# brown-palm/goal-force

Measured on AMD Instinct MI355X. Metric: frames_per_sec (81-frame video / (50-step denoise loop + VAE decode), Wan2.2-I2V-A14B 832x480x81f), higher is better.
Workload: dtype bf16

## Files before the change

### goal_force_amd/csrc/gf_attention.hip

```cpp
#include "gf_common.h"
#include <cstdlib>
#include <type_traits>

namespace {

constexpr int QB = 256;
constexpr int KVB = 64;
constexpr int HD = 128;
constexpr int KV_TILE_BYTES = KVB * HD * 2;

constexpr int K3_RING = 2;
constexpr int K3_DMA0 = 10;
constexpr int K3_DMAS = 8;

struct AttnArgs {
    const u16* q;
    const u16* k;
    const u16* v;
    u16* o;
    int q_len, kv_len, heads, n_qblocks;
    long q_stride, k_stride, v_stride, o_stride;
    float scale_log2e;
    unsigned long long* dbg;
    float* lse;
    const u16* vt;
    long kv_pad;
    float last_key_bias;
};

constexpr int AT2_THREADS = 512;
constexpr int AT2_V_BASE = 2 * KV_TILE_BYTES;
constexpr int AT2_LDS = 4 * KV_TILE_BYTES;

template <int I, int N, class F>
__device__ __forceinline__ void static_for(F&& f) {
    if constexpr (I < N) {
        f(std::integral_constant<int, I>{});
        static_for<I + 1, N>(f);
    }
}
__device__ __forceinline__ void mfma32(f32x16& acc, const bf16x8& a, const bf16x8& b) {
    acc = __builtin_amdgcn_mfma_f32_32x32x16_bf16(a, b, acc, 0, 0, 0);
}

template <bool VT>
__global__ __launch_bounds__(AT2_THREADS, 2) void flash_attn_fwd_kernel2(const AttnArgs p) {
    extern __shared__ __attribute__((aligned(16))) char smem[];
    GF_LDS char* lds = (GF_LDS char*)smem;
    const int tid = threadIdx.x;
    const int lane = tid & 63;
    const int wave = __builtin_amdgcn_readfirstlane(tid >> 6);
    const int r = lane & 31, h = lane >> 5;
    int head, qb;
    {
        const int pid = blockIdx.x;
        if ((p.heads & 7) == 0) {
            const int xcd = pid & 7, idx = pid >> 3;
            head = xcd + 8 * (idx / p.n_qblocks);
            qb = idx % p.n_qblocks;
        } else {
            head = pid / p.n_qblocks;
            qb = pid % p.n_qblocks;
        }
    }
    const int q0 = qb * QB + wave * 32;

    bf16x8 qf[8];
    {
        const int qr = min(q0 + r, p.q_len - 1);
        const u16* qp = p.q + (long)qr * p.q_stride + head * HD + 8 * h;
#pragma unroll
        for (int kd = 0; kd < 8; ++kd) qf[kd] = *reinterpret_cast<const bf16x8*>(qp + 16 * kd);
    }

    const int dma_r = lane >> 4;
    unsigned dma_off[2][2];
#pragma unroll
    for (int jj = 0; jj < 2; ++jj) {
        const int j = 2 * wave + jj;
        const int row = 4 * j + dma_r;
        const int lch = (lane & 15) ^ ((dma_r << 2) | (j & 3));
        dma_off[jj][0] = (unsigned)row * (unsigned)p.k_stride + head * HD + lch * 8;
        dma_off[jj][1] = (unsigned)row * (unsigned)p.v_stride + head * HD + lch * 8;
    }
    const unsigned kstep = KVB * (unsigned)p.k_stride, vstep = KVB * (unsigned)p.v_stride;
    auto dma16 = [&](const u16* g, GF_LDS char* l) {
        unsigned keep;
        const unsigned dst = __builtin_amdgcn_readfirstlane((unsigned)(unsigned long)l);
        asm volatile("s_mov_b32 %0, m0\n\ts_mov_b32 m0, %2\n\ts_nop 0\n\tglobal_load_lds_dwordx4 %1, off\n\ts_mov_b32 m0, %0"
                     : "=&s"(keep)
                     : "v"(g), "s"(dst)
                     : "memory");
    };
    typedef __attribute__((ext_vector_type(4))) unsigned u32x4s;
    auto make_srd = [](const void* base) {
        const unsigned long b = (unsigned long)base;
        u32x4s r;
        r[0] = (unsigned)b;
        r[1] = (unsigned)(b >> 32) & 0xffffu;
        r[2] = 0xffffffffu;
        r[3] = 0x00020000u;
        return r;
    };
    const u32x4s srd_k = make_srd(p.k), srd_v = make_srd(VT ? (const void*)p.vt : (const void*)p.v);
    auto dma16b = [&](const u32x4s& srd, unsigned voff_bytes, unsigned soff_bytes, GF_LDS char* l) {
        unsigned keep;
        const unsigned dst = __builtin_amdgcn_readfirstlane((unsigned)(unsigned long)l);
        asm volatile("s_mov_b32 %0, m0\n\ts_mov_b32 m0, %3\n\ts_nop 0\n\tbuffer_load_dwordx4 %1, %2, %4 offen lds\n\ts_mov_b32 m0, %0"
                     : "=&s"(keep)
                     : "v"(voff_bytes), "s"(srd), "s"(dst), "s"(soff_bytes)
// ... 286 lines not shown
        __syncthreads();
    };

    stage(0, 0, 0);
    if (nt > 1) stage(0, 1, 1);
    asm volatile("s_waitcnt vmcnt(0)" ::: "memory");
    __syncthreads();
    qk_plain(C0{});
    __syncthreads();
    if (nt > 2) stage(0, 2, 0);
    stage(1, 0, 0);
    if (nt > 1) qk_plain(C1{});
    softmax_plain(C0{}, 0);
    asm volatile("s_waitcnt vmcnt(0)" ::: "memory");
    __syncthreads();
    int pi = 1;
    for (; pi + 1 <= nt - 2; pi += 2) {
        phase(C1{}, pi);
        phase(C0{}, pi + 1);
    }
    if (pi <= nt - 2) {
        phase(C1{}, pi);
        ++pi;
    }
    if (nt >= 2) {
        const int par = (nt - 1) & 1;
        stage(1, nt - 1, par);
        apply_pending();
        if (par) {
            pv_plain(C0{});
            softmax_plain(C1{}, nt - 1);
        } else {
            pv_plain(C1{});
            softmax_plain(C0{}, nt - 1);
        }
        asm volatile("s_waitcnt vmcnt(0)" ::: "memory");
        __syncthreads();
    }
    apply_pending();
    if ((nt - 1) & 1)
        pv_plain(C1{});
    else
        pv_plain(C0{});

    {
        const float l_tot = l_run + __shfl_xor(l_run, 32);
        const float inv = 1.0f / l_tot;
        const int qrow = q0 + r;
        if (p.lse && h == 0 && qrow < p.q_len) p.lse[(long)qrow * p.heads + head] = m_run * c + __builtin_amdgcn_logf(l_tot);
        __syncthreads();
        GF_LDS char* ob = lds + wave * 8192;
#pragma unroll
        for (int d = 0; d < 4; ++d)
#pragma unroll
            for (int rg = 0; rg < 4; ++rg) {
                u32x2 pk;
                pk[0] = pack2bf(oacc[d][4 * rg + 0] * inv, oacc[d][4 * rg + 1] * inv);
                pk[1] = pack2bf(oacc[d][4 * rg + 2] * inv, oacc[d][4 * rg + 3] * inv);
                *(GF_LDS u32x2*)(ob + r * 256 + (((4 * d + rg) ^ (r & 15)) << 4) + 8 * h) = pk;
            }
        asm volatile("s_waitcnt lgkmcnt(0)" ::: "memory");
#pragma unroll
        for (int it = 0; it < 8; ++it) {
            const int row = 4 * it + (lane >> 4), ch = lane & 15;
            const u16x8 v8 = *(GF_LDS u16x8*)(ob + row * 256 + ((ch ^ (row & 15)) << 4));
            if (q0 + row < p.q_len)
                *reinterpret_cast<u16x8*>(p.o + (long)(q0 + row) * p.o_stride + head * HD + 8 * ch) = v8;
        }
    }
}

constexpr int K3_NQ = 2;
template <int NQ> struct At3 {
    static constexpr int WAVES = 16 / NQ, THREADS = 64 * WAVES, ROWS = 16 * NQ, PIECES = NQ;
    static constexpr int SLOTS = 32 * NQ;
};
constexpr int AT3_V_BASE = 2 * KV_TILE_BYTES;
constexpr int AT3_LDS = 4 * KV_TILE_BYTES;

__device__ __forceinline__ void mfma16(f32x4& acc, const bf16x8& a, const bf16x8& b) {
    acc = __builtin_amdgcn_mfma_f32_16x16x32_bf16(a, b, acc, 0, 0, 0);
}

template <int NQ>
__global__ __launch_bounds__(At3<NQ>::THREADS, (NQ == 2 ? 2 : 1)) void flash_attn_fwd_kernel3(const AttnArgs p) {
    constexpr int NP = At3<NQ>::PIECES, NW = At3<NQ>::WAVES, RW = At3<NQ>::ROWS, NS = At3<NQ>::SLOTS;
    extern __shared__ __attribute__((aligned(16))) char smem[];
    GF_LDS char* lds = (GF_LDS char*)smem;
    const int tid = threadIdx.x;
    const int lane = tid & 63;
    const int wave = __builtin_amdgcn_readfirstlane(tid >> 6);
    const int r = lane & 15, g = lane >> 4;
    int head, qb0;
    {
        const int pid = blockIdx.x;
        if ((p.heads & 7) == 0) {
            const int xcd = pid & 7, idx = pid >> 3;
            head = xcd + 8 * (idx / p.n_qblocks);
            qb0 = idx % p.n_qblocks;
        } else {
            head = pid / p.n_qblocks;
            qb0 = pid % p.n_qblocks;
        }
    }
    const int q0 = qb0 * QB + wave * RW;

    bf16x8 qf[NQ][4];
#pragma unroll
    for (int qb = 0; qb < NQ; ++qb) {
        const int qr = min(q0 + 16 * qb + r, p.q_len - 1);
        const u16* qp = p.q + (long)qr * p.q_stride + head * HD + 8 * g;
#pragma unroll
        for (int ks = 0; ks < 4; ++ks) {
            qf[qb][ks] = *reinterpret_cast<const bf16x8*>(qp + 32 * ks);
        }
    }

    const int dma_r = lane >> 4;
    unsigned k_off0, vt_off0;
    {
        const int row = 4 * wave + dma_r;
        const int lch = (lane & 15) ^ (row & 15);
        k_off0 = ((unsigned)row * (unsigned)p.k_stride + head * HD + lch * 8) * 2u;
        const int vrow = 8 * wave + (lane >> 3);
        const int vch = (lane & 7) ^ ((vrow >> 1) & 7);
        vt_off0 = (unsigned)(((long)head * HD + vrow) * p.kv_pad + vch * 8) * 2u;
    }
    const unsigned kstep = KVB * (unsigned)p.k_stride * 2u;
    const unsigned k_piece = 4u * NW * (unsigned)p.k_stride * 2u, vt_piece = 8u * NW * (unsigned)p.kv_pad * 2u;
    typedef __attribute__((ext_vector_type(4))) unsigned u32x4s;
    auto make_srd = [](const void* base) {
        const unsigned long b = (unsigned long)base;
        u32x4s s;
        s[0] = (unsigned)b;
        s[1] = (unsigned)(b >> 32) & 0xffffu;
        s[2] = 0xffffffffu;
        s[3] = 0x00020000u;
        return s;
    };
    const u32x4s srd_v = make_srd(p.vt);
    auto dma16b = [&](const u32x4s& srd, unsigned voff_bytes, unsigned soff_bytes, GF_LDS char* l) __attribute__((always_inline)) {
        const unsigned dst = __builtin_amdgcn_readfirstlane((unsigned)(unsigned long)l);
        asm volatile("s_mov_b32 m0, %2\n\ts_nop 0\n\tbuffer_load_dwordx4 %0, %1, %3 offen lds"
                     :
                     : "v"(voff_bytes), "s"(srd), "s"(dst), "s"(soff_bytes)
                     : "memory");
    };
    auto srd_k_tile = [&](int t) __attribute__((always_inline)) {
        const unsigned long bb = (unsigned long)p.k + (unsigned long)(unsigned)t * kstep;
        const int rem = p.kv_len - t * KVB;
        u32x4s sd;
        sd[0] = (unsigned)bb;
        sd[1] = (unsigned)(bb >> 32) & 0xffffu;
        sd[2] = rem > 0 ? (unsigned)rem * (unsigned)p.k_stride * 2u : 0u;
        sd[3] = 0x00020000u;
        return sd;
    };
    auto stage_piece = [&](int which, int t, int buf, int jj) __attribute__((always_inline)) {
        GF_LDS char* base = lds + which * AT3_V_BASE + buf * KV_TILE_BYTES + (NW * jj + wave) * 1024;
        if (which)
            dma16b(srd_v, vt_off0, (unsigned)t * (KVB * 2u) + (unsigned)jj * vt_piece, base);
        else
            dma16b(srd_k_tile(t), k_off0, (unsigned)jj * k_piece, base);
    };
    auto stage = [&](int which, int t, int buf) __attribute__((always_inline)) {
#pragma unroll
        for (int jj = 0; jj < NP; ++jj) stage_piece(which, t, buf, jj);
    };
// ... 152 lines not shown
        if constexpr (F < 16) {
            constexpr int kk = F >> 3, db = F & 7;
            fr[F % RING] = *(GF_LDS bf16x8*)(lds + voff[kk] + db * 2048 + (1 - PAR) * KV_TILE_BYTES);
        } else if constexpr (F < 32) {
            constexpr int ks = (F - 16) >> 2, kb = (F - 16) & 3;
            fr[F % RING] = *(GF_LDS bf16x8*)(lds + koff[ks] + kb * 4096 + (1 - PAR) * KV_TILE_BYTES);
        }
    };
    auto mfma_op = [&](auto s_c, auto par_c) __attribute__((always_inline)) {
        constexpr int S = decltype(s_c)::value, PAR = decltype(par_c)::value;
        constexpr int F = S / NQ, qb = (F & 1) ? NQ - 1 - S % NQ : S % NQ;
        if constexpr (F < 16) {
            constexpr int kk = F >> 3, db = F & 7;
            mfma_pv(oacc[db][qb], fr[F % RING], pf(kk, qb));
        } else {
            constexpr int ks = (F - 16) >> 2, kb = (F - 16) & 3;
            if constexpr (ks == 0) {
                mfma_qk_first(sc[1 - PAR][kb][qb], fr[F % RING], qf[qb][ks], negm[qb]);
            } else {
                mfma_qk(sc[1 - PAR][kb][qb], fr[F % RING], qf[qb][ks]);
            }
        }
    };
    auto dma_slot = [&](auto s_c, auto par_c, int pidx) __attribute__((always_inline)) {
        constexpr int S = decltype(s_c)::value, PAR = decltype(par_c)::value;
        if constexpr (S >= K3_DMA0 && (S - K3_DMA0) % K3_DMAS == 0 && (S - K3_DMA0) / K3_DMAS < 2 * NP) {
            constexpr int i = (S - K3_DMA0) / K3_DMAS;
            if constexpr (i < NP) {
                stage_piece(1, pidx, PAR, i);
            } else {
                stage_piece(0, pidx + 2, PAR, i - NP);
            }
        }
    };
    auto phase = [&](auto par_c, int pidx) __attribute__((always_inline)) {
        constexpr int PAR = decltype(par_c)::value;
        apply_pending();
        static_for<0, RING - 1>([&](auto f_c) { frag_load(f_c, par_c); });
        float mx[NQ];
#pragma unroll
        for (int qb = 0; qb < NQ; ++qb) mx[qb] = -INFINITY;
        static_for<0, 4 * NQ>([&](auto s_c) {
            constexpr int S = decltype(s_c)::value;
            mfma_op(s_c, par_c);
            if constexpr (S % NQ == 0) frag_load(std::integral_constant<int, S / NQ + RING - 1>{}, par_c);
            {
                constexpr int kb = S / NQ, qb = S % NQ;
                const f32x4& v = sc[PAR][kb][qb];
                mx[qb] = fmaxf(fmaxf(mx[qb], v[0]), v[1]);
                mx[qb] = fmaxf(fmaxf(mx[qb], v[2]), v[3]);
            }
            __builtin_amdgcn_sched_barrier(0);
        });
        new_max(par_c, mx, false);
        float pe[2];
        static_for<4 * NQ, NS>([&](auto s_c) {
            constexpr int S = decltype(s_c)::value;
            mfma_op(s_c, par_c);
            if constexpr (S == 8 * NQ - 1 || S == 16 * NQ - 1) {
#pragma unroll
                for (int qb = 0; qb < NQ; ++qb) mfma_pv(oacc[NDB - 1][qb], ones, pf(S / (8 * NQ), qb));
            }
            if constexpr (S % NQ == 0) frag_load(std::integral_constant<int, S / NQ + RING - 1>{}, par_c);
            dma_slot(s_c, par_c, pidx);
            if constexpr (S >= 8 * NQ) {
                constexpr int T = (S - 8 * NQ) % 3, e = ((S - 8 * NQ) / 3) * 2 + (T == 2 ? 1 : T);
                constexpr int kk = e / (8 * NQ), qb = (e >> 3) % NQ, kb = 2 * kk + ((e >> 2) & 1), j = e & 3;
                if constexpr (T != 2) {
                    asm volatile("v_exp_f32 %0, %1" : "=v"(pe[T]) : "v"(sc[PAR][kb][qb][j]));
                } else {
                    unsigned w;
                    asm volatile("v_cvt_pk_bf16_f32 %0, %1, %2" : "=v"(w) : "v"(pe[0]), "v"(pe[1]));
                    pfw[kk][qb][(kb & 1) * 2 + (j >> 1)] = w;
                }
            }
            __builtin_amdgcn_sched_barrier(0);
        });
        asm volatile("s_waitcnt vmcnt(0)" ::: "memory");
        __syncthreads();
    };

    stage(0, 0, 0);
    if (nt > 1) stage(0, 1, 1);
#pragma unroll
    for (int qb = 0; qb < NQ; ++qb)
#pragma unroll
        for (int ks = 0; ks < 4; ++ks)
#pragma unroll
            for (int e = 0; e < 8; ++e) qf[qb][ks][e] = (__bf16)((float)qf[qb][ks][e] * p.scale_log2e);
    asm volatile("s_waitcnt vmcnt(0)" ::: "memory");
    __syncthreads();
    qk_plain(C0{});
    __syncthreads();
    if (nt > 2) stage(0, 2, 0);
    stage(1, 0, 0);
    softmax_plain(C0{}, 0);
    if (nt > 1) qk_plain(C1{});
    asm volatile("s_waitcnt vmcnt(0)" ::: "memory");
    __syncthreads();
    int pi = 1;
    for (; pi + 1 <= nt - 2; pi += 2) {
        phase(C1{}, pi);
        phase(C0{}, pi + 1);
    }
    if (pi <= nt - 2) {
        phase(C1{}, pi);
        ++pi;
    }
    if (nt >= 2) {
        const int par = (nt - 1) & 1;
        stage(1, nt - 1, par);
        apply_pending();
        if (par) {
            pv_plain(C0{});
            softmax_plain(C1{}, nt - 1);
        } else {
            pv_plain(C1{});
            softmax_plain(C0{}, nt - 1);
        }
        asm volatile("s_waitcnt vmcnt(0)" ::: "memory");
        __syncthreads();
    }
    apply_pending();
    if ((nt - 1) & 1)
        pv_plain(C1{});
    else
        pv_plain(C0{});

    {
        float inv[NQ];
#pragma unroll
        for (int qb = 0; qb < NQ; ++qb) {
            const float l = __shfl(oacc[NDB - 1][qb][0], r);
            inv[qb] = 1.0f / l;
            const int qrow = q0 + 16 * qb + r;
            if (p.lse && g == 0 && qrow < p.q_len) p.lse[(long)qrow * p.heads + head] = -negm[qb][0] + __builtin_amdgcn_logf(l);
        }
        __syncthreads();
        GF_LDS char* ob = lds + wave * (RW * 256);
#pragma unroll
        for (int qb = 0; qb < NQ; ++qb)
#pragma unroll
            for (int db = 0; db < 8; ++db) {
                u32x2 pk;
                pk[0] = pack2bf(oacc[db][qb][0] * inv[qb], oacc[db][qb][1] * inv[qb]);
                pk[1] = pack2bf(oacc[db][qb][2] * inv[qb], oacc[db][qb][3] * inv[qb]);
                const int row = 16 * qb + r;
                *(GF_LDS u32x2*)(ob + row * 256 + (((2 * db + (g >> 1)) ^ (row & 15)) << 4) + 8 * (g & 1)) = pk;
            }
        asm volatile("s_waitcnt lgkmcnt(0)" ::: "memory");
#pragma unroll
        for (int it = 0; it < RW / 4; ++it) {
            const int row = 4 * it + (lane >> 4), ch = lane & 15;
            const u16x8 v8 = *(GF_LDS u16x8*)(ob + row * 256 + ((ch ^ (row & 15)) << 4));
            if (q0 + row < p.q_len)
                *reinterpret_cast<u16x8*>(p.o + (long)(q0 + row) * p.o_stride + head * HD + 8 * ch) = v8;
        }
    }
}

__global__ __launch_bounds__(256) void transpose_v32_kernel(const u16* __restrict__ v, u16* __restrict__ vt, int kv_len, long kv_pad,
                                                            long v_stride) {
    __shared__ u16 tile[KVB][HD + 8];
    const int t0 = blockIdx.x * KVB, head = blockIdx.y, tid = threadIdx.x;
#pragma unroll
    for (int it = 0; it < 4; ++it) {
// ... 96 lines not shown
    a.n_qblocks = (int)((q_len + QB - 1) / QB);
    a.q_stride = q_stride;
    a.k_stride = k_stride;
    a.v_stride = v_stride;
    a.o_stride = o_stride;
    a.scale_log2e = scale * 1.4426950408889634f;
    a.lse = lse;
    a.vt = (const u16*)vt;
    a.kv_pad = kv_pad;
    a.last_key_bias = 0.f;
    if (last_key_multiplicity != 1.0f) {
        GF_CHECK_ARG(last_key_multiplicity >= 1.0f && !vt && scale > 0.f,
                     "gf_flash_attn_fwd_lastmult: multiplicity >= 1, plain-V form only (not the V^T form)");
        a.last_key_bias = log2f(last_key_multiplicity) / a.scale_log2e;
    }
    a.dbg = nullptr;
    if (vt)
        hipLaunchKernelGGL(flash_attn_fwd_kernel2<true>, dim3((unsigned)(a.n_qblocks * a.heads)), dim3(AT2_THREADS), AT2_LDS,
                           (hipStream_t)stream, a);
    else
        hipLaunchKernelGGL(flash_attn_fwd_kernel2<false>, dim3((unsigned)(a.n_qblocks * a.heads)), dim3(AT2_THREADS), AT2_LDS,
                           (hipStream_t)stream, a);
    GF_CHECK_LAUNCH("gf_flash_attn_fwd");
    return GF_OK;
}

extern "C" GF_API int gf_flash_attn_fwd(const void* q, const void* k, const void* v, void* o, int64_t q_len, int64_t kv_len,
                                 int64_t heads, int64_t head_dim, int64_t q_stride, int64_t k_stride,
                                 int64_t v_stride, int64_t o_stride, float scale, void* stream) {
    return flash_attn_fwd_impl(q, k, v, o, nullptr, q_len, kv_len, heads, head_dim, q_stride, k_stride, v_stride, o_stride, scale,
                               stream);
}

extern "C" GF_API int gf_flash_attn_fwd_lastmult(const void* q, const void* k, const void* v, void* o, int64_t q_len, int64_t kv_len,
                                                  int64_t heads, int64_t head_dim, int64_t q_stride, int64_t k_stride, int64_t v_stride,
                                                  int64_t o_stride, float scale, float last_key_multiplicity, void* stream) {
    return flash_attn_fwd_impl(q, k, v, o, nullptr, q_len, kv_len, heads, head_dim, q_stride, k_stride, v_stride, o_stride, scale,
                               stream, nullptr, 0, last_key_multiplicity);
}

extern "C" GF_API int gf_flash_attn_fwd_lse(const void* q, const void* k, const void* v, void* o, float* lse, int64_t q_len,
                                     int64_t kv_len, int64_t heads, int64_t head_dim, int64_t q_stride, int64_t k_stride,
                                     int64_t v_stride, int64_t o_stride, float scale, void* stream) {
    GF_CHECK_ARG(lse, "gf_flash_attn_fwd_lse: null lse");
    return flash_attn_fwd_impl(q, k, v, o, lse, q_len, kv_len, heads, head_dim, q_stride, k_stride, v_stride, o_stride, scale,
                               stream);
}

extern "C" GF_API int gf_transpose_v(const void* v, int64_t v_stride, void* vt, int64_t kv_len, int64_t kv_pad, int64_t heads,
                                     void* stream) {
    GF_CHECK_ARG(v && vt, "gf_transpose_v: null pointer");
    GF_CHECK_ARG(kv_len > 0 && heads > 0 && kv_pad >= kv_len && kv_pad % KVB == 0 && v_stride % 8 == 0 && v_stride >= heads * HD,
                 "gf_transpose_v: kv_pad must be a multiple of 64 covering kv_len; v_stride must cover heads*128");
    GF_CHECK_ARG(gf_aligned16(v) && gf_aligned16(vt), "gf_transpose_v: 16-byte alignment required");
    GF_CHECK_ARG(heads * HD * kv_pad < (1LL << 31), "gf_transpose_v: heads*128*kv_pad must stay below 2^31 elements");
    hipLaunchKernelGGL(transpose_v_kernel, dim3((unsigned)(kv_pad / KVB), (unsigned)heads), dim3(256), 0, (hipStream_t)stream,
                       (const u16*)v, (u16*)vt, (int)kv_len, (long)kv_pad, (long)v_stride);
    GF_CHECK_LAUNCH("gf_transpose_v");
    return GF_OK;
}

extern "C" GF_API int gf_flash_attn_fwd_vt(const void* q, const void* k, const void* vt, void* o, float* lse, int64_t q_len,
                                           int64_t kv_len, int64_t kv_pad, int64_t heads, int64_t head_dim, int64_t q_stride,
                                           int64_t k_stride, int64_t o_stride, float scale, void* stream) {
    GF_CHECK_ARG(vt && kv_pad >= kv_len && kv_pad % KVB == 0 && gf_aligned16(vt), "gf_flash_attn_fwd_vt: bad V^T buffer");
    GF_CHECK_ARG(heads * HD * kv_pad < (1LL << 31), "gf_flash_attn_fwd_vt: heads*128*kv_pad must stay below 2^31 elements");
    return flash_attn_fwd_impl(q, k, k, o, lse, q_len, kv_len, heads, head_dim, q_stride, k_stride, k_stride, o_stride, scale,
                               stream, vt, kv_pad);
}

extern "C" GF_API int gf_transpose_v32(const void* v, int64_t v_stride, void* vt, int64_t kv_len, int64_t kv_pad, int64_t heads,
                                       void* stream) {
    GF_CHECK_ARG(v && vt, "gf_transpose_v32: null pointer");
    GF_CHECK_ARG(kv_len > 0 && heads > 0 && kv_pad >= kv_len && kv_pad % KVB == 0 && v_stride % 8 == 0 && v_stride >= heads * HD,
                 "gf_transpose_v32: kv_pad must be a multiple of 64 covering kv_len; v_stride must cover heads*128");
    GF_CHECK_ARG(gf_aligned16(v) && gf_aligned16(vt), "gf_transpose_v32: 16-byte alignment required");
    GF_CHECK_ARG(heads * HD * kv_pad < (1LL << 31), "gf_transpose_v32: heads*128*kv_pad must stay below 2^31 elements");
    hipLaunchKernelGGL(transpose_v32_kernel, dim3((unsigned)(kv_pad / KVB), (unsigned)heads), dim3(256), 0, (hipStream_t)stream,
                       (const u16*)v, (u16*)vt, (int)kv_len, (long)kv_pad, (long)v_stride);
    GF_CHECK_LAUNCH("gf_transpose_v32");
    return GF_OK;
}

extern "C" GF_API int gf_flash_attn_fwd_vt32(const void* q, const void* k, const void* vt, void* o, float* lse, int64_t q_len,
                                             int64_t kv_len, int64_t kv_pad, int64_t heads, int64_t head_dim, int64_t q_stride,
                                             int64_t k_stride, int64_t o_stride, float scale, void* stream) {
    GF_CHECK_ARG(q && k && vt && o, "gf_flash_attn_fwd_vt32: null pointer");
    if (head_dim != HD) {
        gf_set_error("gf_flash_attn_fwd_vt32: head_dim=%ld unsupported (kernel is built for 128)", (long)head_dim);
        return GF_ERR_UNSUPPORTED;
    }
    GF_CHECK_ARG(q_len >= 0 && kv_len >= 2 * KVB && heads > 0 && q_len < (1 << 30) && kv_len < (1 << 30),
                 "gf_flash_attn_fwd_vt32: bad lengths q=%ld kv=%ld heads=%ld (kv_len >= 128)", (long)q_len, (long)kv_len, (long)heads);
    GF_CHECK_ARG(kv_pad >= kv_len && kv_pad % KVB == 0 && heads * HD * kv_pad < (1LL << 31), "gf_flash_attn_fwd_vt32: bad V^T buffer");
    GF_CHECK_ARG(q_stride % 8 == 0 && k_stride % 8 == 0 && o_stride % 4 == 0 && q_stride >= heads * HD && k_stride >= heads * HD &&
                     o_stride >= heads * HD,
                 "gf_flash_attn_fwd_vt32: strides must cover heads*128 and be multiples of 8");
    GF_CHECK_ARG(gf_aligned16(q) && gf_aligned16(k) && gf_aligned16(vt) && gf_aligned16(o),
                 "gf_flash_attn_fwd_vt32: 16-byte alignment required");
    GF_CHECK_ARG((kv_len + 64) * k_stride < (1LL << 31), "gf_flash_attn_fwd_vt32: kv_len*stride must stay below 2^31 elements");
    if (q_len == 0) return GF_OK;
    static GfDeviceOnce once;
    hipError_t e = gf_once_per_device(once, [] {
        return hipFuncSetAttribute(reinterpret_cast<const void*>(flash_attn_fwd_kernel3<K3_NQ>),
                                   hipFuncAttributeMaxDynamicSharedMemorySize, AT3_LDS);
    });
    if (e != hipSuccess) {
        gf_set_error("gf_flash_attn_fwd_vt32: hipFuncSetAttribute failed: %s", hipGetErrorString(e));
        return GF_ERR_LAUNCH;
    }
    AttnArgs a;
    a.q = (const u16*)q;
    a.k = (const u16*)k;
    a.v = (const u16*)k;
    a.o = (u16*)o;
    a.q_len = (int)q_len;
    a.kv_len = (int)kv_len;
    a.heads = (int)heads;
    a.n_qblocks = (int)((q_len + QB - 1) / QB);
    a.q_stride = q_stride;
    a.k_stride = k_stride;
    a.v_stride = k_stride;
    a.o_stride = o_stride;
    a.scale_log2e = scale * 1.4426950408889634f;
    a.lse = lse;
    a.vt = (const u16*)vt;
    a.kv_pad = kv_pad;
    a.dbg = nullptr;
    a.last_key_bias = 0.f;
    hipLaunchKernelGGL(flash_attn_fwd_kernel3<K3_NQ>, dim3((unsigned)(a.n_qblocks * a.heads)), dim3(At3<K3_NQ>::THREADS), AT3_LDS,
                       (hipStream_t)stream, a);
    GF_CHECK_LAUNCH("gf_flash_attn_fwd_vt32");
    return GF_OK;
}
```

### goal_force_amd/csrc/gf_cross_fold.hip

```cpp
#include "gf_common.h"

namespace {

constexpr int CF_HD = 128;
constexpr int CF_MAXK = 64;
constexpr int CF_THREADS = 256;
constexpr int CF_QB = 128;

__device__ __forceinline__ void cf_mfma32(f32x16& acc, const bf16x8& a, const bf16x8& b) {
    acc = __builtin_amdgcn_mfma_f32_32x32x16_bf16(a, b, acc, 0, 0, 0);
}

__global__ __launch_bounds__(CF_THREADS) void cross_probs_kernel(const u16* __restrict__ q, const u16* __restrict__ k, u16* __restrict__ pout,
                                                                 int q_len, int n_keys, int n_pad, int heads, long q_stride, long k_stride,
                                                                 long p_stride, float c, float last_key_bias) {
    __shared__ __attribute__((aligned(16))) char lds[CF_MAXK * 256];
    const int tid = threadIdx.x;
    const int lane = tid & 63, wave = tid >> 6;
    const int r = lane & 31, h = lane >> 5;
    const int head = blockIdx.y;
    const int q0 = blockIdx.x * CF_QB + wave * 32;
    const int halves = n_keys > 32 ? 2 : 1;

#pragma unroll
    for (int i = 0; i < (CF_MAXK * 16) / CF_THREADS; ++i) {
        const int idx = tid + CF_THREADS * i;
        const int row = idx >> 4, ch = idx & 15;
        u16x8 v8 = {0, 0, 0, 0, 0, 0, 0, 0};
        if (row < n_keys) v8 = *reinterpret_cast<const u16x8*>(k + (long)row * k_stride + head * CF_HD + ch * 8);
        const int sk = ((row & 3) << 2) | ((row >> 2) & 3);
        *(u16x8*)(lds + row * 256 + ((ch ^ sk) << 4)) = v8;
    }

    bf16x8 qf[8];
    {
        const int qr = min(q0 + r, q_len - 1);
        const u16* qp = q + (long)qr * q_stride + head * CF_HD + 8 * h;
#pragma unroll
        for (int kd = 0; kd < 8; ++kd) qf[kd] = *reinterpret_cast<const bf16x8*>(qp + 16 * kd);
    }
    __syncthreads();

    f32x16 sc[2];
#pragma unroll
    for (int e = 0; e < 16; ++e) {
        sc[0][e] = 0.f;
        sc[1][e] = 0.f;
    }
    const int sK = ((r & 3) << 2) | ((r >> 2) & 3);
#pragma unroll
    for (int kd = 0; kd < 8; ++kd) {
        const int off = 256 * r + 16 * ((2 * kd + h) ^ sK);
        cf_mfma32(sc[0], *(const bf16x8*)(lds + off), qf[kd]);
        if (halves == 2) cf_mfma32(sc[1], *(const bf16x8*)(lds + off + 32 * 256), qf[kd]);
    }

#pragma unroll
    for (int e = 0; e < 16; ++e) {
        const int key = 4 * h + (e & 3) + 8 * (e >> 2);
        if (key >= n_keys) sc[0][e] = -INFINITY;
        if (key + 32 >= n_keys) sc[1][e] = -INFINITY;
        if (key == n_keys - 1) sc[0][e] += last_key_bias;
        if (key + 32 == n_keys - 1) sc[1][e] += last_key_bias;
    }
    float mx = sc[0][0];
#pragma unroll
    for (int e = 1; e < 16; ++e) mx = fmaxf(mx, sc[0][e]);
#pragma unroll
    for (int e = 0; e < 16; ++e) mx = fmaxf(mx, sc[1][e]);
    mx = fmaxf(mx, __shfl_xor(mx, 32));
    const float mc = mx * c;
    float rs = 0.f;
#pragma unroll
    for (int e = 0; e < 16; ++e) {
        sc[0][e] = __builtin_amdgcn_exp2f(__builtin_fmaf(sc[0][e], c, -mc));
        sc[1][e] = __builtin_amdgcn_exp2f(__builtin_fmaf(sc[1][e], c, -mc));
        rs += sc[0][e] + sc[1][e];
    }
    const float l_tot = rs + __shfl_xor(rs, 32);
    const float inv = 1.0f / l_tot;
    float pl = 0.f;
#pragma unroll
    for (int e = 0; e < 16; ++e) {
        const int key = 4 * h + (e & 3) + 8 * (e >> 2);
        if (key == n_keys - 1) pl = sc[0][e];
        if (key + 32 == n_keys - 1) pl = sc[1][e];
    }
    pl += __shfl_xor(pl, 32);
    const float wl = pl * inv;
    const float wl_lo = wl - bf2f(f2bf(wl));

    const int qrow = q0 + r;
    if (qrow < q_len) {
        u16* prow = pout + (long)qrow * p_stride + (long)head * n_pad;
#pragma unroll
        for (int half = 0; half < 2; ++half)
#pragma unroll
            for (int g = 0; g < 4; ++g) {
                const int key = 32 * half + 8 * g + 4 * h;
                if (key < n_pad) {
                    float w4[4];
#pragma unroll
                    for (int i = 0; i < 4; ++i) w4[i] = key + i == n_keys ? wl_lo : sc[half][4 * g + i] * inv;
                    u32x2 pk;
                    pk[0] = pack2bf(w4[0], w4[1]);
                    pk[1] = pack2bf(w4[2], w4[3]);
                    *reinterpret_cast<u32x2*>(prow + key) = pk;
                }
            }
    }
}

constexpr int CFT_ROWS = 64;
__global__ __launch_bounds__(CF_THREADS) void cross_fold_table_kernel(const u16* __restrict__ v, const u16* __restrict__ w, u16* __restrict__ u,
                                                                      int n_keys, int n_pad, int n_out, long v_stride, long w_stride,
                                                                      long u_stride) {
    __shared__ __attribute__((aligned(16))) u16 vs[CF_MAXK * CF_HD];
    const int tid = threadIdx.x;
    const int head = blockIdx.y;
    for (int idx = tid; idx < n_pad * 16; idx += CF_THREADS) {
        const int row = idx >> 4, ch = idx & 15;
        u16x8 v8 = {0, 0, 0, 0, 0, 0, 0, 0};
        if (row <= n_keys) v8 = *reinterpret_cast<const u16x8*>(v + (long)min(row, n_keys - 1) * v_stride + head * CF_HD + ch * 8);
        *reinterpret_cast<u16x8*>(vs + row * CF_HD + ch * 8) = v8;
    }
    __syncthreads();
    const int n = blockIdx.x * CFT_ROWS + (tid >> 2), jg = tid & 3;
    if (n >= n_out) return;
    const int nj = n_pad >> 2;
    float acc[CF_MAXK / 4];
#pragma unroll
    for (int i = 0; i < CF_MAXK / 4; ++i) acc[i] = 0.f;
    const u16* wr = w + (long)n * w_stride + head * CF_HD;
    for (int d0 = 0; d0 < CF_HD; d0 += 8) {
        const u16x8 w8 = *reinterpret_cast<const u16x8*>(wr + d0);
        float wf[8];
#pragma unroll
        for (int e = 0; e < 8; ++e) wf[e] = bf2f(w8[e]);
#pragma unroll
        for (int i = 0; i < CF_MAXK / 4; ++i) {
            if (i < nj) {
                const u16x8 v8 = *reinterpret_cast<const u16x8*>(vs + (jg + 4 * i) * CF_HD + d0);
#pragma unroll
                for (int e = 0; e < 8; ++e) acc[i] = __builtin_fmaf(bf2f(v8[e]), wf[e], acc[i]);
            }
        }
    }
    u16* ur = u + (long)n * u_stride + (long)head * n_pad;
#pragma unroll
    for (int i = 0; i < CF_MAXK / 4; ++i) {
        const int j = jg + 4 * i;
        if (i < nj) ur[j] = j <= n_keys ? f2bf(acc[i]) : (u16)0;
    }
}

}

extern "C" GF_API int gf_cross_probs(const void* q, const void* k, void* p, int64_t q_len, int64_t n_keys, int64_t n_pad, int64_t heads,
                                     int64_t head_dim, int64_t q_stride, int64_t k_stride, int64_t p_stride, float scale,
                                     float last_key_multiplicity, void* stream) {
    GF_CHECK_ARG(q && k && p, "gf_cross_probs: null pointer");
    if (head_dim != CF_HD) {
        gf_set_error("gf_cross_probs: head_dim=%ld unsupported (kernel is built for 128)", (long)head_dim);
        return GF_ERR_UNSUPPORTED;
    }
    GF_CHECK_ARG(q_len >= 0 && q_len < (1 << 30) && heads > 0 && heads < 65536, "gf_cross_probs: bad sizes q=%ld heads=%ld", (long)q_len,
                 (long)heads);
    GF_CHECK_ARG(n_keys >= 1 && n_pad % 16 == 0 && n_pad > n_keys && n_pad <= CF_MAXK,
                 "gf_cross_probs: 1 <= n_keys=%ld < n_pad=%ld <= 64, n_pad a multiple of 16", (long)n_keys, (long)n_pad);
    GF_CHECK_ARG(q_stride % 8 == 0 && k_stride % 8 == 0 && p_stride % 4 == 0 && q_stride >= heads * CF_HD && k_stride >= heads * CF_HD &&
                     p_stride >= heads * n_pad,
                 "gf_cross_probs: strides must cover the rows (q, k: multiples of 8; p: of 4, >= heads * n_pad)");
    GF_CHECK_ARG(gf_aligned16(q) && gf_aligned16(k) && ((uintptr_t)p & 7u) == 0, "gf_cross_probs: alignment (q, k 16 bytes, p 8 bytes)");
    GF_CHECK_ARG(scale > 0.f && last_key_multiplicity >= 1.0f, "gf_cross_probs: scale > 0, multiplicity >= 1");
    if (q_len == 0) return GF_OK;
    const float c = scale * 1.4426950408889634f;
    const float bias = last_key_multiplicity != 1.0f ? log2f(last_key_multiplicity) / c : 0.f;
    const dim3 grid((unsigned)((q_len + CF_QB - 1) / CF_QB), (unsigned)heads);
    hipLaunchKernelGGL(cross_probs_kernel, grid, dim3(CF_THREADS), 0, (hipStream_t)stream, (const u16*)q, (const u16*)k, (u16*)p,
                       (int)q_len, (int)n_keys, (int)n_pad, (int)heads, (long)q_stride, (long)k_stride, (long)p_stride, c, bias);
    GF_CHECK_LAUNCH("gf_cross_probs");
    return GF_OK;
}

extern "C" GF_API int gf_cross_fold_table(const void* v, const void* w_o, void* u, int64_t n_keys, int64_t n_pad, int64_t heads,
                                          int64_t head_dim, int64_t n_out, int64_t v_stride, int64_t w_stride, int64_t u_stride,
                                          void* stream) {
    GF_CHECK_ARG(v && w_o && u, "gf_cross_fold_table: null pointer");
    if (head_dim != CF_HD) {
        gf_set_error("gf_cross_fold_table: head_dim=%ld unsupported (kernel is built for 128)", (long)head_dim);
        return GF_ERR_UNSUPPORTED;
    }
    GF_CHECK_ARG(heads > 0 && heads < 65536 && n_out > 0 && n_out < (1 << 30), "gf_cross_fold_table: bad sizes heads=%ld N=%ld", (long)heads,
                 (long)n_out);
    GF_CHECK_ARG(n_keys >= 1 && n_pad % 16 == 0 && n_pad > n_keys && n_pad <= CF_MAXK,
                 "gf_cross_fold_table: 1 <= n_keys=%ld < n_pad=%ld <= 64, n_pad a multiple of 16", (long)n_keys, (long)n_pad);
    GF_CHECK_ARG(v_stride % 8 == 0 && w_stride % 8 == 0 && v_stride >= heads * CF_HD && w_stride >= heads * CF_HD && u_stride >= heads * n_pad,
                 "gf_cross_fold_table: strides must cover the rows (v, w_o: multiples of 8; u >= heads * n_pad)");
    GF_CHECK_ARG(gf_aligned16(v) && gf_aligned16(w_o) && ((uintptr_t)u & 1u) == 0, "gf_cross_fold_table: alignment");
    const dim3 grid((unsigned)((n_out + CFT_ROWS - 1) / CFT_ROWS), (unsigned)heads);
    hipLaunchKernelGGL(cross_fold_table_kernel, grid, dim3(CF_THREADS), 0, (hipStream_t)stream, (const u16*)v, (const u16*)w_o, (u16*)u,
                       (int)n_keys, (int)n_pad, (int)n_out, (long)v_stride, (long)w_stride, (long)u_stride);
    GF_CHECK_LAUNCH("gf_cross_fold_table");
    return GF_OK;
}
```

### goal_force_amd/csrc/gf_gemm.hip

```cpp
#include "gf_common.h"
#include <cstdlib>
#include <type_traits>


namespace {

constexpr int BM = 256, BN = 256, BK = 64;
constexpr int GEMM_THREADS = 512;
constexpr int TILE_BYTES = BM * BK * 2;
constexpr int STAGE_BYTES = 2 * TILE_BYTES;
constexpr int GEMM_LDS = 2 * STAGE_BYTES;
constexpr int GROUP_M = 8;

struct ConvGeom {
    const u16* src;
    const u16* cache;
    const u16* zero;
    int H, W, C, Ho, Wo, kt, ks, mode, t_stride, t_off, taps;
    int hist_front;
    int c64;
    long frame;
    float inv_c, inv_ks2;
};

struct GemmArgs {
    const u16* A;
    const u16* W;
    const u16* bias;
    u16* C;
    const u16* R;
    const u16* gate;
    const float* row_scale;
    int M, N, K;
    long lda, ldw, ldc, ldr;
    long sA = 0, sW = 0, sC = 0;
    int tiles_m, tiles_n;
    unsigned long long* rsv0 = nullptr;
    ConvGeom cv;
    int rsv1 = 0;
    int stagger;
    int wrows;
    int stagger_rows;
    int group_m;
    int rsv2 = 0;
};

constexpr int GF_EPI_VT32 = 6;

__device__ __forceinline__ void glds16(const void* g, GF_LDS char* l) {
    __builtin_amdgcn_global_load_lds((const GF_GLOBAL void*)g, (GF_LDS void*)l, 16, 0, 0);
}

typedef __attribute__((ext_vector_type(8))) int i32x8;

template <int EPI>
__device__ __forceinline__ float gf_epi_act(float lin) {
    if constexpr (EPI == GF_EPI_BIAS_GELU_TANH) return gelu_tanh_f(rbf(lin));
    else if constexpr (EPI == GF_EPI_BIAS_SILU) {
        const float y = rbf(lin);
        return y / (1.0f + expf(-y));
    } else return lin;
}

template <int EPI, bool FP8>
__global__ __launch_bounds__(GEMM_THREADS, 2) void gemm_kernel(const GemmArgs p) {
    static_assert(FP8, "only the fp8 form of this kernel ships (launch_gemm); bf16 with M < 512 runs gemm_ph_kernel");
    constexpr int ESZ = FP8 ? 1 : 2;
    constexpr int BKE = 128 / ESZ;
    extern __shared__ __attribute__((aligned(16))) char smem[];
    GF_LDS char* lds = (GF_LDS char*)smem;

    const int tid = threadIdx.x;
    const int lane = tid & 63;
    const int wave = __builtin_amdgcn_readfirstlane(tid >> 6);

    const int nwg = p.tiles_m * p.tiles_n;
    int v;
    {
        const int pid = blockIdx.x;
        const int xcd = pid & 7, local = pid >> 3;
        const int q = nwg >> 3, r = nwg & 7;
        v = (xcd < r ? xcd * (q + 1) : r * (q + 1) + (xcd - r) * q) + local;
    }
    const int per_group = GROUP_M * p.tiles_n;
    const int group = v / per_group;
    const int first_m = group * GROUP_M;
    const int gsz = min(p.tiles_m - first_m, GROUP_M);
    const int in_group = v - group * per_group;
    const int tile_m = first_m + in_group % gsz;
    const int tile_n = in_group / gsz;
    const int m0 = tile_m * BM, n0 = tile_n * BN;

    const int srow = lane >> 3;
    const int schunk = (lane & 7) ^ srow;
    const char* a_src[4];
    const char* b_src[4];
#pragma unroll
    for (int i = 0; i < 4; ++i) {
        const int row = (wave * 4 + i) * 8 + srow;
        const int am = min(m0 + row, p.M - 1);
        const int bn = min(n0 + row, p.N - 1);
        a_src[i] = (const char*)p.A + ((long)am * p.lda) * ESZ + schunk * 16;
        b_src[i] = (const char*)p.W + ((long)bn * p.ldw) * ESZ + schunk * 16;
    }
    auto stage = [&](int buf, int kt) {
        GF_LDS char* sa = lds + buf * STAGE_BYTES + wave * 4096;
        GF_LDS char* sb = sa + TILE_BYTES;
        const int koff = kt * 128;
#pragma unroll
        for (int i = 0; i < 4; ++i) {
            glds16(a_src[i] + koff, sa + i * 1024);
            glds16(b_src[i] + koff, sb + i * 1024);
        }
    };

    const int wm = wave >> 2, wn = wave & 3;
    const int frow = lane & 15;
    const int fq = lane >> 4;
    const int sw = frow & 7;
    const int a_base = (wm * 128 + frow) * 128;
    const int b_base = TILE_BYTES + (wn * 64 + frow) * 128;
    const int ch0 = ((0 * 4 + fq) ^ sw) << 4;
    const int ch1 = ((1 * 4 + fq) ^ sw) << 4;

    f32x4 acc[8][4];
#pragma unroll
    for (int i = 0; i < 8; ++i)
#pragma unroll
        for (int j = 0; j < 4; ++j) acc[i][j] = f32x4{0.f, 0.f, 0.f, 0.f};

// ... 605 lines not shown
#pragma unroll
        for (int it = 0; it < 32; ++it) {
            const int mr = m0 + wm * 128 + it * 4 + (lane >> 4);
            if (mr < p.M && nr < p.N) {
                rres[it] = __builtin_nontemporal_load(reinterpret_cast<const u16x8*>(p.R + (long)mr * p.ldr + nr));
            } else {
                rres[it] = u16x8{0, 0, 0, 0, 0, 0, 0, 0};
            }
        }
    }
    f32x4 csc[(FP8 && EPI == GF_EPI_VT32) ? 8 : 1];
    if constexpr (FP8 && EPI == GF_EPI_VT32) {
#pragma unroll
        for (int j = 0; j < 8; ++j) {
            const int n = n0 + wn * 128 + j * 16 + fq * 4;
#pragma unroll
            for (int r = 0; r < 4; ++r) csc[j][r] = (n + r < p.wrows) ? p.row_scale[n + r] : 0.f;
        }
    }
    a4_static_for<0, 8>([&](auto j_c) {
        constexpr int j = decltype(j_c)::value;
        const int n = n0 + wn * 128 + j * 16 + fq * 4;
        const float bv[4] = {bf2f(bpre[j][0]), bf2f(bpre[j][1]), bf2f(bpre[j][2]), bf2f(bpre[j][3])};
        a4_static_for<0, 8>([&](auto i_c) {
            constexpr int i = decltype(i_c)::value;
            constexpr int A0 = (i * 8 + j) * 4;
            float y[4] = {a4_acc<A0>(), a4_acc<A0 + 1>(), a4_acc<A0 + 2>(), a4_acc<A0 + 3>()};
            if constexpr (FP8 && EPI != GF_EPI_VT32) {
#pragma unroll
                for (int r = 0; r < 4; ++r) y[r] = y[r] * rsc[i] + bv[r];
            }
            if constexpr (EPI == GF_EPI_VT32) {
                const float bm = bf2f(bpre[i][0]);
                if constexpr (FP8) {
#pragma unroll
                    for (int r = 0; r < 4; ++r) y[r] = (n + r < p.wrows) ? y[r] * csc[j][r] + bm : 0.f;
                } else {
#pragma unroll
                    for (int r = 0; r < 4; ++r) y[r] = (n + r < p.wrows) ? y[r] + bm : 0.f;
                }
            } else if constexpr (EPI == GF_EPI_BIAS_GELU_TANH) {
                const unsigned l01 = FP8 ? pack2bf(y[0], y[1]) : pack2bf(y[0] + bv[0], y[1] + bv[1]);
                const unsigned l23 = FP8 ? pack2bf(y[2], y[3]) : pack2bf(y[2] + bv[2], y[3] + bv[3]);
                gf_f32x2 g01 = {__uint_as_float(l01 << 16), __uint_as_float(l01 & 0xffff0000u)};
                gf_f32x2 g23 = {__uint_as_float(l23 << 16), __uint_as_float(l23 & 0xffff0000u)};
                gelu_tanh_f4(g01, g23);
                y[0] = g01[0];
                y[1] = g01[1];
                y[2] = g23[0];
                y[3] = g23[1];
            } else {
#pragma unroll
                for (int r = 0; r < 4; ++r) {
                    y[r] = gf_epi_act<EPI>(FP8 ? y[r] : y[r] + bv[r]);
                }
            }
            u32x2 pk;
            pk[0] = pack2bf(y[0], y[1]);
            pk[1] = pack2bf(y[2], y[3]);
            const int row = i * 16 + frow;
            const int slot = (j * 4 + fq) ^ ((row & 15) << 1);
            *(GF_LDS u32x2*)(ep + row * 256 + slot * 8) = pk;
        });
    });
    asm volatile("s_waitcnt lgkmcnt(0)" ::: "memory");
    {
        const int cc = lane & 15;
        const int n = n0 + wn * 128 + cc * 8;
        const bool n_ok = n < p.N;
        const u16x8 g8 = gpre;
#pragma unroll
        for (int it = 0; it < 32; ++it) {
            const int row = it * 4 + (lane >> 4);
            const int m = m0 + wm * 128 + row;
            u16x8 yv;
            if constexpr (EPI == GF_EPI_VT32) {
                const int G = cc >> 2, g = cc & 3, sw = (row & 15) << 1;
                const u16x4 lo = *(GF_LDS u16x4*)(ep + row * 256 + (((8 * G + g) ^ sw) << 3));
                const u16x4 hi = *(GF_LDS u16x4*)(ep + row * 256 + (((8 * G + 4 + g) ^ sw) << 3));
                yv = u16x8{lo[0], lo[1], lo[2], lo[3], hi[0], hi[1], hi[2], hi[3]};
            } else {
                yv = *(GF_LDS u16x8*)(ep + row * 256 + ((cc ^ (row & 15)) << 4));
            }
            if (m < p.M && n_ok) {
                u16x8 o = yv;
                if constexpr (HAS_R) {
                    const u16x8 r8 = rres[it];
#pragma unroll
                    for (int e = 0; e < 8; ++e) {
                        float t = bf2f(yv[e]);
                        if (EPI == GF_EPI_BIAS_GATE_RESID) t = rbf(bf2f(g8[e]) * t);
                        o[e] = (EPI == GF_EPI_BIAS_MUL) ? f2bf(t * bf2f(r8[e]))
                                                        : f2bf(bf2f(r8[e]) + t);
                    }
                }
                __builtin_nontemporal_store(o, reinterpret_cast<u16x8*>(p.C + (long)m * p.ldc + n));
            }
        }
    }
}

template <int EPI, bool FP8 = false>
int launch_gemm_a4(const GemmArgs& a0, hipStream_t stream) {
    GemmArgs a = a0;
    {
        const int g = gf_options().a4_group_m.load(std::memory_order_relaxed);
        a.group_m = g > 0 ? g : (a.K * (FP8 ? 1 : 2) >= 16384 ? 4 : GROUP_M);
    }
    static GfDeviceOnce once;
    hipError_t e = gf_once_per_device(once, [] {
        return hipFuncSetAttribute(reinterpret_cast<const void*>(gemm_a4_kernel<EPI, FP8>),
                                   hipFuncAttributeMaxDynamicSharedMemorySize, GEMM_LDS);
    });
    if (e != hipSuccess) {
        gf_set_error("gf_gemm: hipFuncSetAttribute(%d B LDS) failed: %s", GEMM_LDS, hipGetErrorString(e));
        return GF_ERR_LAUNCH;
    }
    hipLaunchKernelGGL((gemm_a4_kernel<EPI, FP8>), dim3((unsigned)(a.tiles_m * a.tiles_n)), dim3(A4_THREADS), GEMM_LDS, stream, a);
    GF_CHECK_LAUNCH(FP8 ? "gf_gemm_fp8" : "gf_gemm_bf16");
    return GF_OK;
}

template <int EPI, bool FP8>
int launch_gemm(const GemmArgs& a, hipStream_t stream) {
    const bool use_a4 = gf_options().prefer_8wave.load(std::memory_order_relaxed) == 0;
    if constexpr (!FP8) {
        if (use_a4 && a.M >= 512 && a.K % 64 == 0 && 256L * a.lda * 2 + a.K * 2L < (1L << 31) &&
            256L * a.ldw * 2 + a.K * 2L < (1L << 31))
            return launch_gemm_a4<EPI>(a, stream);
    } else {
        if (use_a4 && a.M >= 512 && a.K % 128 == 0 && 256L * a.lda + a.K < (1L << 31) && 256L * a.ldw + a.K < (1L << 31))
            return launch_gemm_a4<EPI, true>(a, stream);
    }
    static GfDeviceOnce once;
    hipError_t e = gf_once_per_device(once, [] {
        const void* fn;
        if constexpr (FP8) fn = reinterpret_cast<const void*>(gemm_kernel<EPI, true>);
        else fn = reinterpret_cast<const void*>(gemm_ph_kernel<EPI, false>);
        return hipFuncSetAttribute(fn, hipFuncAttributeMaxDynamicSharedMemorySize, GEMM_LDS);
    });
    if (e != hipSuccess) {
        gf_set_error("gf_gemm: hipFuncSetAttribute(%d B LDS) failed: %s", GEMM_LDS, hipGetErrorString(e));
        return GF_ERR_LAUNCH;
    }
    if constexpr (FP8)
        hipLaunchKernelGGL((gemm_kernel<EPI, true>), dim3((unsigned)(a.tiles_m * a.tiles_n)), dim3(GEMM_THREADS), GEMM_LDS, stream, a);
    else
        hipLaunchKernelGGL((gemm_ph_kernel<EPI, false>), dim3((unsigned)(a.tiles_m * a.tiles_n)), dim3(GEMM_THREADS), GEMM_LDS,
                           stream, a);
    GF_CHECK_LAUNCH(FP8 ? "gf_gemm_fp8" : "gf_gemm_bf16");
    return GF_OK;
}

template <int EPI, int NB, int CONV>
int launch_conv(const GemmArgs& a, hipStream_t stream, int batch = 1) {
    static GfDeviceOnce once;
    hipError_t e = gf_once_per_device(once, [] {
        return hipFuncSetAttribute(reinterpret_cast<const void*>(gemm_ph_kernel<EPI, false, CONV, NB>),
                                   hipFuncAttributeMaxDynamicSharedMemorySize, GEMM_LDS);
    });
    if (e != hipSuccess) {
        gf_set_error("gf_conv3d: hipFuncSetAttribute(%d B LDS) failed: %s", GEMM_LDS, hipGetErrorString(e));
        return GF_ERR_LAUNCH;
    }
    hipLaunchKernelGGL((gemm_ph_kernel<EPI, false, CONV, NB>), dim3((unsigned)(a.tiles_m * a.tiles_n), (unsigned)batch), dim3(GEMM_THREADS),
                       GEMM_LDS, stream, a);
    GF_CHECK_LAUNCH("gf_conv3d_bf16");
    return GF_OK;
}

}
__device__ __attribute__((used, visibility("default"))) u16 gf_conv_zero_page[128] = {};
namespace {

const u16* conv_zero_page() {
    static GfDeviceOnce once;
    static const u16* page[64] = {};
    int dev = 0;
    if (hipGetDevice(&dev) != hipSuccess || dev < 0 || dev >= 64) return nullptr;
    hipError_t e = gf_once_per_device(once, [dev] {
        void* z = nullptr;
        hipError_t r = hipGetSymbolAddress(&z, HIP_SYMBOL(gf_conv_zero_page));
        if (r == hipSuccess) page[dev] = (const u16*)z;
        return r;
    });
    return e == hipSuccess ? page[dev] : nullptr;
}

}

static int gemm_dispatch(bool fp8, const void* A, int64_t lda, const void* W, int64_t ldw, const float* row_scale,
                         const void* bias, void* C, int64_t ldc, int64_t M, int64_t N, int64_t K, int epilogue,
                         const void* resid, int64_t ldr, const void* gate, void* stream) {
    const char* fn = fp8 ? "gf_gemm_fp8" : "gf_gemm_bf16";
    const int bke = fp8 ? 128 : 64, lal = fp8 ? 16 : 8;
    GF_CHECK_ARG(A && W && C, "%s: null A/W/C", fn);
    GF_CHECK_ARG(M >= 0 && N > 0 && K > 0, "%s: bad sizes M=%ld N=%ld K=%ld", fn, (long)M, (long)N, (long)K);
    GF_CHECK_ARG(K % bke == 0, "%s: K=%ld must be a multiple of %d", fn, (long)K, bke);
    GF_CHECK_ARG(N % 8 == 0, "%s: N=%ld must be a multiple of 8", fn, (long)N);
    GF_CHECK_ARG(lda % lal == 0 && ldw % lal == 0 && ldc % 8 == 0 && lda >= K && ldw >= K && ldc >= N,
                 "%s: leading dimensions must be multiples of %d (A/W) / 8 (C) and cover the row", fn, lal);
    GF_CHECK_ARG(gf_aligned16(A) && gf_aligned16(W) && gf_aligned16(C) && (!bias || gf_aligned16(bias)),
                 "%s: 16-byte alignment required", fn);
    GF_CHECK_ARG(M < (1 << 30) && N < (1 << 30), "%s: M/N too large", fn);
    GF_CHECK_ARG(!fp8 || row_scale, "%s: row_scale is required", fn);
    const bool need_r = epilogue == GF_EPI_BIAS_GATE_RESID || epilogue == GF_EPI_BIAS_RESID || epilogue == GF_EPI_BIAS_MUL;
    GF_CHECK_ARG(!need_r || (resid && ldr % 8 == 0 && ldr >= N && gf_aligned16(resid)),
                 "%s: residual epilogue needs an aligned resid with ldr >= N", fn);
    GF_CHECK_ARG(epilogue != GF_EPI_BIAS_GATE_RESID || (gate && gf_aligned16(gate)),
                 "%s: gate epilogue needs an aligned gate vector", fn);
    if (M == 0) return GF_OK;
    GemmArgs a;
    a.A = (const u16*)A;
    a.W = (const u16*)W;
    a.bias = (const u16*)bias;
    a.C = (u16*)C;
    a.R = (const u16*)resid;
    a.gate = (const u16*)gate;
    a.row_scale = row_scale;
    a.M = (int)M;
    a.N = (int)N;
    a.K = (int)K;
    a.lda = lda;
    a.ldw = ldw;
    a.ldc = ldc;
    a.ldr = ldr;
    a.tiles_m = (int)((M + BM - 1) / BM);
    a.tiles_n = (int)((N + BN - 1) / BN);
    a.stagger = gf_options().a4_stagger.load(std::memory_order_relaxed);
    a.wrows = (int)N;
    a.stagger_rows = 0;
    hipStream_t s = (hipStream_t)stream;
#define GF_GEMM_CASE(E) case E: return fp8 ? launch_gemm<E, true>(a, s) : launch_gemm<E, false>(a, s);
    switch (epilogue) {
        GF_GEMM_CASE(GF_EPI_BIAS)
        GF_GEMM_CASE(GF_EPI_BIAS_GELU_TANH)
        GF_GEMM_CASE(GF_EPI_BIAS_GATE_RESID)
        GF_GEMM_CASE(GF_EPI_BIAS_RESID)
        GF_GEMM_CASE(GF_EPI_BIAS_SILU)
        GF_GEMM_CASE(GF_EPI_BIAS_MUL)
        default:
            gf_set_error("%s: unknown epilogue %d", fn, epilogue);
            return GF_ERR_INVALID_ARG;
    }
#undef GF_GEMM_CASE
}

extern "C" GF_API int gf_gemm_bf16(const void* A, int64_t lda, const void* W, int64_t ldw, const void* bias, void* C,
                                   int64_t ldc, int64_t M, int64_t N, int64_t K, int epilogue, const void* resid,
                                   int64_t ldr, const void* gate, void* stream) {
    return gemm_dispatch(false, A, lda, W, ldw, nullptr, bias, C, ldc, M, N, K, epilogue, resid, ldr, gate, stream);
}

extern "C" GF_API int gf_gemm_fp8(const void* A8, int64_t lda, const void* W8, int64_t ldw, const float* row_scale,
                                  const void* bias, void* C, int64_t ldc, int64_t M, int64_t N, int64_t K, int epilogue,
                                  const void* resid, int64_t ldr, const void* gate, void* stream) {
    return gemm_dispatch(true, A8, lda, W8, ldw, row_scale, bias, C, ldc, M, N, K, epilogue, resid, ldr, gate, stream);
}

extern "C" GF_API int gf_linear_vt32(const void* x, int64_t ldx, const void* w, int64_t ldw, const void* bias, void* vt,
                                     int64_t kv_len, int64_t kv_pad, int64_t N, int64_t K, void* stream) {
    GF_CHECK_ARG(x && w && vt, "gf_linear_vt32: null x/w/vt");
    GF_CHECK_ARG(kv_len > 0 && kv_pad >= kv_len && kv_pad % 64 == 0 && kv_pad - kv_len < 64, "gf_linear_vt32: kv_pad = kv_len rounded up to 64");
    GF_CHECK_ARG(N >= 512 && N % 128 == 0 && K > 0 && K % 64 == 0, "gf_linear_vt32: N=%ld (>= 512, multiple of 128), K=%ld (multiple of 64)", (long)N, (long)K);
    GF_CHECK_ARG(ldx % 8 == 0 && ldw % 8 == 0 && ldx >= K && ldw >= K, "gf_linear_vt32: leading dimensions must be multiples of 8 covering K");
    GF_CHECK_ARG(gf_aligned16(x) && gf_aligned16(w) && gf_aligned16(vt) && (!bias || ((uintptr_t)bias & 1u) == 0), "gf_linear_vt32: alignment");
    GF_CHECK_ARG(N * kv_pad < (1LL << 31) && 256L * ldx * 2 + K * 2L < (1L << 31) && 256L * ldw * 2 + K * 2L < (1L << 31),
                 "gf_linear_vt32: operand too large for 32-bit staging offsets");
    GemmArgs a;
    a.A = (const u16*)w;
    a.W = (const u16*)x;
    a.bias = (const u16*)bias;
    a.C = (u16*)vt;
    a.R = nullptr;
    a.gate = nullptr;
    a.row_scale = nullptr;
    a.M = (int)N;
    a.N = (int)kv_pad;
    a.K = (int)K;
    a.lda = ldw;
    a.ldw = ldx;
    a.ldc = kv_pad;
    a.ldr = 0;
    a.tiles_m = (int)((N + BM - 1) / BM);
    a.tiles_n = (int)((kv_pad + BN - 1) / BN);
    a.stagger = gf_options().a4_stagger.load(std::memory_order_relaxed);
    a.wrows = (int)kv_len;
    a.stagger_rows = 1;
    return launch_gemm_a4<GF_EPI_VT32>(a, (hipStream_t)stream);
}

extern "C" GF_API int gf_linear_vt32_fp8(const void* x8, int64_t ldx, const float* x_scale, const void* w8, int64_t ldw, const void* bias,
                                         void* vt, int64_t kv_len, int64_t kv_pad, int64_t N, int64_t K, void* stream) {
    GF_CHECK_ARG(x8 && w8 && vt && x_scale, "gf_linear_vt32_fp8: null x8/w8/vt/x_scale");
    GF_CHECK_ARG(kv_len > 0 && kv_pad >= kv_len && kv_pad % 64 == 0 && kv_pad - kv_len < 64, "gf_linear_vt32_fp8: kv_pad = kv_len rounded up to 64");
    GF_CHECK_ARG(N >= 512 && N % 128 == 0 && K > 0 && K % 128 == 0, "gf_linear_vt32_fp8: N=%ld (>= 512, multiple of 128), K=%ld (multiple of 128)", (long)N, (long)K);
    GF_CHECK_ARG(ldx % 16 == 0 && ldw % 16 == 0 && ldx >= K && ldw >= K, "gf_linear_vt32_fp8: leading dimensions must be multiples of 16 covering K");
    GF_CHECK_ARG(gf_aligned16(x8) && gf_aligned16(w8) && gf_aligned16(vt) && (!bias || ((uintptr_t)bias & 1u) == 0), "gf_linear_vt32_fp8: alignment");
    GF_CHECK_ARG(N * kv_pad < (1LL << 31) && 256L * ldx + K < (1L << 31) && 256L * ldw + K < (1L << 31),
                 "gf_linear_vt32_fp8: operand too large for 32-bit staging offsets");
    GemmArgs a;
    a.A = (const u16*)w8;
    a.W = (const u16*)x8;
    a.bias = (const u16*)bias;
    a.C = (u16*)vt;
    a.R = nullptr;
    a.gate = nullptr;
    a.row_scale = x_scale;
    a.M = (int)N;
    a.N = (int)kv_pad;
    a.K = (int)K;
    a.lda = ldw;
    a.ldw = ldx;
    a.ldc = kv_pad;
    a.ldr = 0;
    a.tiles_m = (int)((N + BM - 1) / BM);
    a.tiles_n = (int)((kv_pad + BN - 1) / BN);
    a.stagger = gf_options().a4_stagger.load(std::memory_order_relaxed);
    a.wrows = (int)kv_len;
    a.stagger_rows = 1;
    return launch_gemm_a4<GF_EPI_VT32, true>(a, (hipStream_t)stream);
}

extern "C" GF_API int gf_gemm_bf16_batched(const void* A, int64_t lda, int64_t strideA, const void* W, int64_t ldw, int64_t strideW,
                                           void* C, int64_t ldc, int64_t strideC, int64_t M, int64_t N, int64_t K, int64_t batch,
                                           void* stream) {
    GF_CHECK_ARG(A && W && C, "gf_gemm_bf16_batched: null A/W/C");
    GF_CHECK_ARG(M > 0 && N > 0 && K > 0 && batch > 0 && batch < 65536, "gf_gemm_bf16_batched: bad sizes");
    GF_CHECK_ARG(K % 64 == 0 && N % 8 == 0, "gf_gemm_bf16_batched: K=%ld must be a multiple of 64 and N=%ld of 8", (long)K, (long)N);
    GF_CHECK_ARG(lda >= K && ldw >= K && ldc >= N && lda % 8 == 0 && ldw % 8 == 0 && ldc % 8 == 0 && strideA % 8 == 0 && strideW % 8 == 0 &&
                     strideC % 8 == 0 && strideA >= 0 && strideW >= 0 && strideC >= 0,
                 "gf_gemm_bf16_batched: leading dimensions / strides must be multiples of 8 elements covering K / N");
    GF_CHECK_ARG(gf_aligned16(A) && gf_aligned16(W) && gf_aligned16(C), "gf_gemm_bf16_batched: 16-byte alignment required");
    GF_CHECK_ARG(M < (1L << 30) && N < (1L << 30), "gf_gemm_bf16_batched: M / N too large");
// ... 127 lines not shown
```

### goal_force_amd/csrc/gf_rowops.hip

```cpp
#include "gf_common.h"

namespace {

constexpr int ROW_THREADS = 128;
constexpr int ROW_NCH = 8;

__global__ __launch_bounds__(ROW_THREADS) void layernorm_modulate_kernel(
    const u16* __restrict__ x, u16* __restrict__ out, const u16* __restrict__ weight,
    const u16* __restrict__ bias, const u16* __restrict__ scale1p, const u16* __restrict__ shift,
    int dim, long x_stride, long out_stride, float eps) {
    __shared__ float red[ROW_THREADS / 64];
    const long row = blockIdx.x;
    const int tid = threadIdx.x;
    const int nchunks = dim >> 3;
    const u16* xr = x + row * x_stride;
    u16x8 v[ROW_NCH];
    float s = 0.f;
#pragma unroll
    for (int i = 0; i < ROW_NCH; ++i) {
        const int c = tid + i * ROW_THREADS;
        if (c < nchunks) {
            v[i] = *reinterpret_cast<const u16x8*>(xr + (c << 3));
#pragma unroll
            for (int j = 0; j < 8; ++j) s += bf2f(v[i][j]);
        }
    }
    const float mean = block_sum<ROW_THREADS>(s, red) / (float)dim;
    float q = 0.f;
#pragma unroll
    for (int i = 0; i < ROW_NCH; ++i) {
        const int c = tid + i * ROW_THREADS;
        if (c < nchunks) {
#pragma unroll
            for (int j = 0; j < 8; ++j) {
                const float d = bf2f(v[i][j]) - mean;
                q += d * d;
            }
        }
    }
    const float var = block_sum<ROW_THREADS>(q, red) / (float)dim;
    const float rstd = 1.0f / sqrtf(var + eps);
    u16* orow = out + row * out_stride;
#pragma unroll
    for (int i = 0; i < ROW_NCH; ++i) {
        const int c = tid + i * ROW_THREADS;
        if (c < nchunks) {
            u16x8 w8, b8, sc8, sh8;
            if (weight) w8 = *reinterpret_cast<const u16x8*>(weight + (c << 3));
            if (bias) b8 = *reinterpret_cast<const u16x8*>(bias + (c << 3));
            if (scale1p) sc8 = *reinterpret_cast<const u16x8*>(scale1p + (c << 3));
            if (shift) sh8 = *reinterpret_cast<const u16x8*>(shift + (c << 3));
            u16x8 o;
#pragma unroll
            for (int j = 0; j < 8; ++j) {
                float y = (bf2f(v[i][j]) - mean) * rstd;
                if (weight) y = y * bf2f(w8[j]);
                if (bias) y = y + bf2f(b8[j]);
                y = rbf(y);
                if (scale1p) y = rbf(y * bf2f(sc8[j]));
                if (shift) y = rbf(y + bf2f(sh8[j]));
                o[j] = f2bf(y);
            }
            *reinterpret_cast<u16x8*>(orow + (c << 3)) = o;
        }
    }
}

__global__ __launch_bounds__(ROW_THREADS) void rmsnorm_rope_kernel(
    u16* __restrict__ x, const u16* __restrict__ weight, const float* __restrict__ cos_tab,
    const float* __restrict__ sin_tab, int dim, int head_dim, long x_stride, float eps) {
    __shared__ float red[ROW_THREADS / 64];
    const long row = blockIdx.x;
    const int tid = threadIdx.x;
    const int nchunks = dim >> 3;
    u16* xr = x + row * x_stride;
    u16x8 v[ROW_NCH];
    float s = 0.f;
#pragma unroll
    for (int i = 0; i < ROW_NCH; ++i) {
        const int c = tid + i * ROW_THREADS;
        if (c < nchunks) {
            v[i] = *reinterpret_cast<const u16x8*>(xr + (c << 3));
#pragma unroll
// ... 179 lines not shown
        const float sc = fmaxf(rbf(mx / 448.0f), 1.0f);
        if (lane == 0) scale_out[row] = sc;
        const float den = sc + 1e-8f;
        const bool unit = den == 1.0f;
        unsigned char* orow = (unsigned char*)outp + row * out_stride + lane * 8;
#pragma unroll
        for (int i = 0; i < NCH; ++i) {
            unsigned w[2];
#pragma unroll
            for (int h2 = 0; h2 < 2; ++h2) {
                gf_f32x2 f0 = unpack2bf(v[i][2 * h2]), f1 = unpack2bf(v[i][2 * h2 + 1]);
                if (!unit) {
                    f0 = gf_f32x2{f0[0] / den, f0[1] / den};
                    f1 = gf_f32x2{f1[0] / den, f1[1] / den};
                }
                unsigned t = 0;
                t = __builtin_amdgcn_cvt_pk_fp8_f32(f0[0], f0[1], t, false);
                t = __builtin_amdgcn_cvt_pk_fp8_f32(f1[0], f1[1], t, true);
                w[h2] = t;
            }
            *reinterpret_cast<u32x2*>(orow + i * 512) = u32x2{w[0], w[1]};
        }
    }
}

template <int NCH, int ROPE>
__global__ __launch_bounds__(64 * WROWS) void rmsnorm_rope_wave_kernel(u16* __restrict__ x, const u16* __restrict__ weight,
                                                                         const float* __restrict__ cos_tab,
                                                                         const float* __restrict__ sin_tab, long rows,
                                                                         int head_dim, long x_stride, float eps) {
    constexpr int DIM = NCH * 512;
    const long row = (long)blockIdx.x * WROWS + (threadIdx.x >> 6);
    if (row >= rows) return;
    const int lane = threadIdx.x & 63;
    u16* xr = x + row * x_stride + lane * 8;
    u16x8 v[NCH];
    float s = 0.f;
#pragma unroll
    for (int i = 0; i < NCH; ++i) {
        v[i] = *reinterpret_cast<const u16x8*>(xr + i * 512);
#pragma unroll
        for (int j = 0; j < 8; ++j) {
            const float f = bf2f(v[i][j]);
            s += f * f;
        }
    }
    const float rstd = 1.0f / sqrtf(wave_sum(s) * (1.0f / DIM) + eps);
    const int half = head_dim >> 1;
    f32x4 cs1 = {0.f, 0.f, 0.f, 0.f}, sn1 = {0.f, 0.f, 0.f, 0.f};
    if constexpr (ROPE == 1) {
        const int p0 = ((lane * 8) % head_dim) >> 1;
        cs1 = *reinterpret_cast<const f32x4*>(cos_tab + row * half + p0);
        sn1 = *reinterpret_cast<const f32x4*>(sin_tab + row * half + p0);
    }
#pragma unroll
    for (int i = 0; i < NCH; ++i) {
        const int c0 = i * 512 + lane * 8;
        const u16x8 w8 = *reinterpret_cast<const u16x8*>(weight + c0);
        float y[8];
#pragma unroll
        for (int j = 0; j < 8; ++j) {
            const float n = rbf(bf2f(v[i][j]) * rstd);
            y[j] = rbf(n * bf2f(w8[j]));
        }
        u16x8 o;
        if constexpr (ROPE != 0) {
            f32x4 cs = cs1, sn = sn1;
            if constexpr (ROPE == 2) {
                const int p0 = (c0 % head_dim) >> 1;
                cs = *reinterpret_cast<const f32x4*>(cos_tab + row * half + p0);
                sn = *reinterpret_cast<const f32x4*>(sin_tab + row * half + p0);
            }
#pragma unroll
            for (int p = 0; p < 4; ++p) {
                const float a = y[2 * p], b = y[2 * p + 1];
                o[2 * p] = f2bf(__builtin_fmaf(a, cs[p], -(b * sn[p])));
                o[2 * p + 1] = f2bf(__builtin_fmaf(a, sn[p], b * cs[p]));
            }
        } else {
#pragma unroll
            for (int j = 0; j < 8; ++j) o[j] = f2bf(y[j]);
        }
        *reinterpret_cast<u16x8*>(xr + i * 512) = o;
    }
}

__global__ __launch_bounds__(ROW_THREADS) void quant_fp8_rowscale_kernel(const u16* __restrict__ x,
                                                                         unsigned char* __restrict__ out,
                                                                         float* __restrict__ scale, int dim,
                                                                         long x_stride, long out_stride) {
    __shared__ float red[ROW_THREADS / 64];
    const long row = blockIdx.x;
    const int tid = threadIdx.x;
    const int nchunks = dim >> 3;
    const u16* xr = x + row * x_stride;
    constexpr int NCH = 14;
    u16x8 v[NCH];
    float mx = 0.f;
#pragma unroll
    for (int i = 0; i < NCH; ++i) {
        const int c = tid + i * ROW_THREADS;
        if (c < nchunks) {
            v[i] = *reinterpret_cast<const u16x8*>(xr + (c << 3));
#pragma unroll
            for (int j = 0; j < 8; ++j) mx = fmaxf(mx, fabsf(bf2f(v[i][j])));
        }
    }
#pragma unroll
    for (int o = 32; o > 0; o >>= 1) mx = fmaxf(mx, __shfl_xor(mx, o));
    if ((tid & 63) == 0) red[tid >> 6] = mx;
    __syncthreads();
    mx = fmaxf(red[0], red[1]);
    const float sc = fmaxf(rbf(mx / 448.0f), 1.0f);
    if (tid == 0) scale[row] = sc;
    const float den = sc + 1e-8f;
    unsigned char* orow = out + row * out_stride;
#pragma unroll
    for (int i = 0; i < NCH; ++i) {
        const int c = tid + i * ROW_THREADS;
        if (c < nchunks) {
            float f[8];
#pragma unroll
            for (int j = 0; j < 8; ++j) f[j] = bf2f(v[i][j]) / den;
            unsigned w0 = 0, w1 = 0;
            w0 = __builtin_amdgcn_cvt_pk_fp8_f32(f[0], f[1], w0, false);
            w0 = __builtin_amdgcn_cvt_pk_fp8_f32(f[2], f[3], w0, true);
            w1 = __builtin_amdgcn_cvt_pk_fp8_f32(f[4], f[5], w1, false);
            w1 = __builtin_amdgcn_cvt_pk_fp8_f32(f[6], f[7], w1, true);
            *reinterpret_cast<u32x2*>(orow + (c << 3)) = u32x2{w0, w1};
        }
    }
}

template <int NCH>
__global__ __launch_bounds__(64 * WROWS) void layernorm_modulate_fp8_wave_kernel(
    const u16* __restrict__ x, unsigned char* __restrict__ out8, float* __restrict__ scale, const u16* __restrict__ weight,
    const u16* __restrict__ bias, const u16* __restrict__ scale1p, const u16* __restrict__ shift, long rows, long x_stride,
    long out_stride, float eps) {
    constexpr int DIM = NCH * 512;
    const long row = (long)blockIdx.x * WROWS + (threadIdx.x >> 6);
    if (row >= rows) return;
    const int lane = threadIdx.x & 63;
    const u16* xr = x + row * x_stride + lane * 8;
    u16x8 v[NCH];
    float s = 0.f;
#pragma unroll
    for (int i = 0; i < NCH; ++i) {
        v[i] = *reinterpret_cast<const u16x8*>(xr + i * 512);
#pragma unroll
        for (int j = 0; j < 8; ++j) s += bf2f(v[i][j]);
    }
    const float mean = wave_sum(s) * (1.0f / DIM);
    float q = 0.f;
#pragma unroll
    for (int i = 0; i < NCH; ++i)
#pragma unroll
        for (int j = 0; j < 8; ++j) {
            const float d = bf2f(v[i][j]) - mean;
            q += d * d;
        }
    const float rstd = 1.0f / sqrtf(wave_sum(q) * (1.0f / DIM) + eps);
    float mx = 0.f;
#pragma unroll
    for (int i = 0; i < NCH; ++i) {
        const int c0 = i * 512 + lane * 8;
        u16x8 w8, b8, sc8, sh8;
// ... 118 lines not shown
    hipLaunchKernelGGL(layernorm_modulate_kernel, dim3((unsigned)rows), dim3(ROW_THREADS), 0,
                       (hipStream_t)stream, (const u16*)x, (u16*)out, (const u16*)weight, (const u16*)bias,
                       (const u16*)scale1p, (const u16*)shift, (int)dim, (long)x_stride, (long)out_stride, eps);
    GF_CHECK_LAUNCH("gf_layernorm_modulate");
    return GF_OK;
}

extern "C" GF_API int gf_layernorm_modulate_fp8(const void* x, void* out8, float* scale, const void* weight, const void* bias,
                                                const void* scale1p, const void* shift, int64_t rows, int64_t dim,
                                                int64_t x_stride, int64_t out_stride, float eps, void* stream) {
    GF_CHECK_ARG(x && out8 && scale, "gf_layernorm_modulate_fp8: null x/out8/scale");
    GF_CHECK_ARG(rows >= 0 && (dim == 5120 || dim == 4096 || dim == 1536),
                 "gf_layernorm_modulate_fp8: dim=%ld is not one of the wave-per-row widths (5120, 4096, 1536); use "
                 "gf_layernorm_modulate + gf_quant_fp8_rowscale", (long)dim);
    GF_CHECK_ARG(x_stride % 8 == 0 && out_stride % 8 == 0 && gf_aligned16(x) && (((uintptr_t)out8) & 7u) == 0,
                 "gf_layernorm_modulate_fp8: rows must be 16-byte (x) / 8-byte (out8) aligned");
    GF_CHECK_ARG((!weight || gf_aligned16(weight)) && (!bias || gf_aligned16(bias)) &&
                     (!scale1p || gf_aligned16(scale1p)) && (!shift || gf_aligned16(shift)),
                 "gf_layernorm_modulate_fp8: vectors must be 16-byte aligned");
    if (rows == 0) return GF_OK;
    {
        const int mode = (!weight && !bias && !scale1p && !shift) ? 0 : (weight && bias && !scale1p && !shift) ? 1
                         : (!weight && !bias && scale1p && shift) ? 2 : -1;
        const void* av = mode == 1 ? weight : scale1p;
        const void* bv = mode == 1 ? bias : shift;
        const dim3 grid_((unsigned)((rows + WROWS - 1) / WROWS)), block_(64 * WROWS);
#define GF_LN2(NCH, M)                                                                                                   \
    if (dim == NCH * 512 && mode == M) {                                                                                 \
        hipLaunchKernelGGL((layernorm_wave2_kernel<NCH, M, true>), grid_, block_, 0, (hipStream_t)stream, (const u16*)x, out8,     \
                           scale, (const u16*)av, (const u16*)bv, (long)rows, (long)x_stride, (long)out_stride, eps);   \
        GF_CHECK_LAUNCH("gf_layernorm_modulate_fp8");                                                                    \
        return GF_OK;                                                                                                    \
    }
        GF_LN2(10, 0) GF_LN2(10, 1) GF_LN2(10, 2) GF_LN2(8, 0) GF_LN2(8, 1) GF_LN2(8, 2) GF_LN2(3, 0) GF_LN2(3, 1) GF_LN2(3, 2)
#undef GF_LN2
    }
#define GF_LN8_WAVE(NCH)                                                                                                 \
    if (dim == NCH * 512) {                                                                                              \
        hipLaunchKernelGGL(layernorm_modulate_fp8_wave_kernel<NCH>, dim3((unsigned)((rows + WROWS - 1) / WROWS)),        \
                           dim3(64 * WROWS), 0, (hipStream_t)stream, (const u16*)x, (unsigned char*)out8, scale,          \
                           (const u16*)weight, (const u16*)bias, (const u16*)scale1p, (const u16*)shift, (long)rows,     \
                           (long)x_stride, (long)out_stride, eps);                                                       \
    }
    GF_LN8_WAVE(10) GF_LN8_WAVE(8) GF_LN8_WAVE(3)
#undef GF_LN8_WAVE
    GF_CHECK_LAUNCH("gf_layernorm_modulate_fp8");
    return GF_OK;
}

extern "C" GF_API int gf_rmsnorm_rope(void* x, const void* weight, const float* cos_tab, const float* sin_tab,
                               int64_t rows, int64_t dim, int64_t head_dim, int64_t x_stride, float eps,
                               void* stream) {
    GF_CHECK_ARG(x && weight, "gf_rmsnorm_rope: null x/weight");
    GF_CHECK_ARG(rows >= 0 && dim > 0 && dim % 8 == 0 && dim <= ROW_THREADS * ROW_NCH * 8,
                 "gf_rmsnorm_rope: dim=%ld must be a multiple of 8 and <= %d", (long)dim,
                 ROW_THREADS * ROW_NCH * 8);
    GF_CHECK_ARG((cos_tab == nullptr) == (sin_tab == nullptr), "gf_rmsnorm_rope: cos/sin must both be set or both NULL");
    GF_CHECK_ARG(head_dim > 0 && head_dim % 8 == 0 && dim % head_dim == 0,
                 "gf_rmsnorm_rope: head_dim=%ld must be a multiple of 8 dividing dim", (long)head_dim);
    GF_CHECK_ARG(x_stride % 8 == 0 && gf_aligned16(x) && gf_aligned16(weight) &&
                     (!cos_tab || (gf_aligned16(cos_tab) && gf_aligned16(sin_tab))),
                 "gf_rmsnorm_rope: 16-byte alignment required");
    if (rows == 0) return GF_OK;
#define GF_RMS_WAVE_ROPE(NCH, ROPE)                                                                                      \
    if (rope_ == ROPE)                                                                                                   \
        hipLaunchKernelGGL((rmsnorm_rope_wave_kernel<NCH, ROPE>), grid_, block_, 0, (hipStream_t)stream, (u16*)x,        \
                           (const u16*)weight, cos_tab, sin_tab, (long)rows, (int)head_dim, (long)x_stride, eps);
#define GF_RMS_WAVE(NCH)                                                                                                 \
    if (dim == NCH * 512) {                                                                                              \
        const dim3 grid_((unsigned)((rows + WROWS - 1) / WROWS)), block_(64 * WROWS);                                     \
        const int rope_ = !cos_tab ? 0 : (512 % head_dim == 0 ? 1 : 2);                                                  \
        GF_RMS_WAVE_ROPE(NCH, 0) GF_RMS_WAVE_ROPE(NCH, 1) GF_RMS_WAVE_ROPE(NCH, 2)                                        \
        GF_CHECK_LAUNCH("gf_rmsnorm_rope");                                                                              \
        return GF_OK;                                                                                                    \
    }
    GF_RMS_WAVE(10) GF_RMS_WAVE(8) GF_RMS_WAVE(3)
#undef GF_RMS_WAVE
#undef GF_RMS_WAVE_ROPE
    hipLaunchKernelGGL(rmsnorm_rope_kernel, dim3((unsigned)rows), dim3(ROW_THREADS), 0, (hipStream_t)stream,
                       (u16*)x, (const u16*)weight, cos_tab, sin_tab, (int)dim, (int)head_dim, (long)x_stride, eps);
    GF_CHECK_LAUNCH("gf_rmsnorm_rope");
    return GF_OK;
}
```

### goal_force_amd/dit.py

```python
from __future__ import annotations

import math
from typing import Optional, Tuple

import torch
import torch.nn as nn

from . import ops
from ._lib import GoalForceError


def precompute_freqs_cis(dim: int, end: int = 1024, theta: float = 10000.0):
    freqs = 1.0 / (theta ** (torch.arange(0, dim, 2)[: (dim // 2)].double() / dim))
    freqs = torch.outer(torch.arange(end), freqs)
    return torch.polar(torch.ones_like(freqs), freqs)


def precompute_freqs_cis_3d(dim: int, end: int = 1024, theta: float = 10000.0):
    return (precompute_freqs_cis(dim - 2 * (dim // 3), end, theta),
            precompute_freqs_cis(dim // 3, end, theta),
            precompute_freqs_cis(dim // 3, end, theta))


class RopeTable:
# ... 29 lines not shown
def _as_rope(freqs, device) -> RopeTable:
    if isinstance(freqs, RopeTable):
        return freqs
    if torch.is_tensor(freqs) and freqs.is_complex():
        return RopeTable(freqs.detach().cpu(), device)
    raise GoalForceError("freqs must be a RopeTable or the reference's complex [S,1,d/2] tensor")


_SINUSOID_FREQS = {}


def sinusoidal_embedding_1d(dim, position):
    key = (dim, position.device)
    inv = _SINUSOID_FREQS.get(key)
    if inv is None:
        inv = torch.pow(10000, -torch.arange(dim // 2, dtype=torch.float64).div(dim // 2)).to(position.device)
        _SINUSOID_FREQS[key] = inv
    sinusoid = torch.outer(position.detach().type(torch.float64), inv)
    return torch.cat([torch.cos(sinusoid), torch.sin(sinusoid)], dim=1).to(position.dtype)


def flash_attention(q: torch.Tensor, k: torch.Tensor, v: torch.Tensor, num_heads: int, compatibility_mode=False):
    if q.dim() != 3 or k.dim() != 3 or v.dim() != 3 or not (q.shape[0] == k.shape[0] == v.shape[0]):
        raise GoalForceError("flash_attention: q, k, v must be [B, S, num_heads * head_dim] with equal B")
    return torch.stack([ops.flash_attn(q[b].contiguous(), k[b].contiguous(), v[b].contiguous(), num_heads, finished_q=True)
                        for b in range(q.shape[0])])


def modulate(x: torch.Tensor, shift: torch.Tensor, scale: torch.Tensor):
    if x.dim() == 2:
        return ops.modulate(x, shift.reshape(-1).contiguous(), scale.reshape(-1).contiguous())
    d = x.shape[-1]
    sh, sc = (t.reshape(-1, d) if t.numel() != d else t.reshape(1, d) for t in (shift, scale))
    if sh.shape[0] not in (1, x.shape[0]) or sc.shape[0] not in (1, x.shape[0]):
        raise GoalForceError("modulate: shift / scale must be [B or 1, 1, D] (per-token modulation is outside the Goal-Force path)")
    return torch.stack([ops.modulate(x[b].contiguous(), sh[b if sh.shape[0] > 1 else 0].contiguous(),
                                     sc[b if sc.shape[0] > 1 else 0].contiguous()) for b in range(x.shape[0])])


def rope_apply(x: torch.Tensor, freqs, num_heads: int):
    rope = _as_rope(freqs, x.device)
    hd = x.shape[-1] // num_heads
    return torch.stack([ops.rope_apply(x[b].contiguous(), rope.cos, rope.sin, hd) for b in range(x.shape[0])])


_CACHE_EPOCH = [0]


def invalidate_caches():
    _CACHE_EPOCH[0] += 1


def param_key(*tensors):
    return (_CACHE_EPOCH[0],) + tuple((id(t), str(t.device), t.data_ptr(), None if t.is_inference() else t._version) for t in tensors)


class QuantizedInput:

    def __init__(self, x2=None, x8=None, scale=None):
        self.x8, self.scale = ops.quant_fp8_rowscale(x2) if x2 is not None else (x8, scale)

    @classmethod
    def layernorm(cls, x2, **kw):
        return cls(None, *ops.layernorm_modulate_fp8(x2, **kw))

    @property
    def shape(self):
        return self.x8.shape

    @property
    def is_cuda(self):
        return self.x8.is_cuda


def linear(x2, lin: nn.Linear, epilogue=ops.EPI_BIAS, resid=None, gate=None, out=None):
    w8 = getattr(lin, "_gf_w8", None)
    if w8 is None:
        return ops.gemm(x2, lin.weight, lin.bias, epilogue=epilogue, resid=resid, gate=gate, out=out)
    if lin._gf_w8_key != param_key(lin.weight):
        w8 = lin._gf_w8 = ops.cast_fp8(lin.weight.detach().contiguous())
        lin._gf_w8_key = param_key(lin.weight)
    q = x2 if isinstance(x2, QuantizedInput) else QuantizedInput(x2)
    return ops.gemm_fp8(q.x8, q.scale, w8, lin.bias, epilogue=epilogue, resid=resid, gate=gate, out=out)


def enable_fp8(module: nn.Module, enabled=True):
    for blk in module.modules():
        if isinstance(blk, DiTBlock):
            for lin in blk.modules():
                if isinstance(lin, nn.Linear):
                    lin._gf_w8 = ops.cast_fp8(lin.weight.detach().contiguous()) if enabled else None
                    lin._gf_w8_key = param_key(lin.weight) if enabled else None
    return module



def enable_sage_attention(module: nn.Module, enabled=True):
    for blk in module.modules():
        if isinstance(blk, DiTBlock):
            blk.self_attn._gf_sage = bool(enabled)
    return module


def sageattn(q, k, v, tensor_layout="HND", is_causal=False, sm_scale=None, return_lse=False, **kw):
    if is_causal:
        raise GoalForceError("sageattn: is_causal=True is not supported (the Wan DiT attention is non-causal)")
    if return_lse:
        raise GoalForceError("sageattn: return_lse=True is not supported")
    if tensor_layout not in ("HND", "NHD"):
        raise GoalForceError(f"sageattn: tensor_layout {tensor_layout!r} (HND or NHD)")
    if q.dim() != 4 or k.dim() != 4 or v.dim() != 4:
        raise GoalForceError("sageattn: q, k, v must be 4-D")
    if q.shape[-1] != 128 or k.shape[-1] != 128 or v.shape[-1] != 128:
        raise GoalForceError(f"sageattn: head_dim {q.shape[-1]} is not supported (the kernel is built for 128)")
    if tensor_layout == "HND":
        q, k, v = (t.transpose(1, 2) for t in (q, k, v))
    B, sq, n, _ = q.shape
    if k.shape[0] != B or v.shape != k.shape or k.shape[2] != n:
        raise GoalForceError("sageattn: q / k / v batch, head or key counts differ")
    out = torch.empty((B, sq, n, 128), dtype=torch.bfloat16, device=q.device)
    for b in range(B):
        q2, k2, v2 = (t[b].reshape(t.shape[1], n * 128) for t in (q, k, v))
        ops.sage_attn(q2, k2, v2, n, scale=sm_scale, out=out[b].view(sq, n * 128))
    return out.transpose(1, 2) if tensor_layout == "HND" else out


def pad_run(ctx2: torch.Tensor) -> int:
    L = ctx2.shape[0]
    if L < 2:
        return max(L - 1, 0)
    differs = (ctx2[1:] != ctx2[:-1]).any(dim=1)
    idx = torch.nonzero(differs)
    return int(idx[-1]) + 1 if idx.numel() else 0


def _tokens2d(x: torch.Tensor) -> torch.Tensor:
    if x.dim() == 3:
        if x.shape[0] != 1:
            raise GoalForceError("hot-path modules take batch 1 ([1,S,D]); loop over the batch")
        return x[0]
    return x


class RMSNorm(nn.Module):

    def __init__(self, dim, eps=1e-5):
        super().__init__()
        self.eps = eps
        self.weight = nn.Parameter(torch.ones(dim))

    def forward(self, x):
        y = x.clone()
        ops.rmsnorm_rope(_tokens2d(y), self.weight, None, None, head_dim=8, eps=self.eps)
        return y


class SelfAttention(nn.Module):

    def __init__(self, dim: int, num_heads: int, eps: float = 1e-6):
        super().__init__()
        self.dim, self.num_heads, self.head_dim = dim, num_heads, dim // num_heads
        self.q, self.k, self.v, self.o = (nn.Linear(dim, dim) for _ in range(4))
        self.norm_q, self.norm_k = RMSNorm(dim, eps=eps), RMSNorm(dim, eps=eps)

    def attend(self, x2: torch.Tensor, rope: RopeTable, sp=None, keep=None) -> torch.Tensor:
        fp8 = getattr(self.q, "_gf_w8", None) is not None
        sage = getattr(self, "_gf_sage", False)
        if sage and keep is not None:
            raise GoalForceError("training through a block with enable_sage_attention is refused (the sage backend has no backward): "
                                 "call enable_sage_attention(module, False) first")
        attn = ops.sage_attn if sage else ops.flash_attn
        xin = (x2 if isinstance(x2, QuantizedInput) else QuantizedInput(x2)) if fp8 else x2
        q_cos, q_sin, attn_scale = rope.cos, rope.sin, None
        if ops._OPT["attn_q_prescale"]:
            (q_cos, q_sin), attn_scale = rope.scaled(Q_PRESCALE(self.head_dim)), math.log(2.0)
        if sp is not None and keep is None:
            k = linear(xin, self.k)
            ops.rmsnorm_rope(k, self.norm_k.weight, rope.cos, rope.sin, self.head_dim, self.norm_k.eps)
            hk = sp.heads_start(k, self.num_heads)
            hv = sp.heads_start(linear(xin, self.v), self.num_heads)
            q = linear(xin, self.q)
            ops.rmsnorm_rope(q, self.norm_q.weight, q_cos, q_sin, self.head_dim, self.norm_q.eps)
            hq = sp.heads_start(q, self.num_heads)
            return sp.attention_started(hq, hk, hv, self.num_heads, tuple(q.shape), scale=attn_scale, backend="sage" if sage else "flash")
        q, k = linear(xin, self.q), linear(xin, self.k)
        if keep is not None and keep.get("wide"):
            keep["qp"], keep["kp"] = q, k
            q, k = q.clone(), k.clone()
        ops.rmsnorm_rope(q, self.norm_q.weight, q_cos, q_sin, self.head_dim, self.norm_q.eps)
        ops.rmsnorm_rope(k, self.norm_k.weight, rope.cos, rope.sin, self.head_dim, self.norm_k.eps)
        if sp is None and keep is None and not fp8 and x2.is_cuda and self.v.weight.shape[0] >= 512 \
                and ops.vt32_ok(x2.shape[0], self.num_heads, self.head_dim):
            return attn(q, k, None, self.num_heads, vt=ops.linear_vt32(x2, self.v.weight, self.v.bias), scale=attn_scale)
        if sp is None and keep is None and fp8 and xin.is_cuda and self.v.weight.shape[0] >= 512 and self.v.weight.shape[1] % 128 == 0 \
                and ops.vt32_ok(xin.shape[0], self.num_heads, self.head_dim):
            if self.v._gf_w8_key != param_key(self.v.weight):
                self.v._gf_w8 = ops.cast_fp8(self.v.weight.detach().contiguous())
                self.v._gf_w8_key = param_key(self.v.weight)
            return attn(q, k, None, self.num_heads, vt=ops.linear_vt32_fp8(xin.x8, xin.scale, self.v._gf_w8, self.v.bias), scale=attn_scale)
        v = linear(xin, self.v)
        if sp is not None:
            return sp.attention(q, k, v, self.num_heads, scale=attn_scale, backend="sage" if sage else "flash")
        if keep is not None:
            keep["attn"], keep["lse"] = ops.flash_attn_lse(q, k, v, self.num_heads, scale=attn_scale)
            if keep.get("wide"):
                keep["v"] = v
            return keep["attn"]
        return attn(q, k, v, self.num_heads, scale=attn_scale)

    def forward(self, x, freqs):
        x2 = _tokens2d(x)
        a = self.attend(x2, _as_rope(freqs, x.device))
        return linear(a, self.o).view(x.shape)


class CrossAttention(nn.Module):

    def __init__(self, dim: int, num_heads: int, eps: float = 1e-6, has_image_input: bool = False):
        super().__init__()
        if has_image_input:
            raise NotImplementedError("has_image_input=True (CLIP image tokens) is outside the Goal-Force path")
        self.dim, self.num_heads, self.head_dim = dim, num_heads, dim // num_heads
        self.q, self.k, self.v, self.o = (nn.Linear(dim, dim) for _ in range(4))
        self.norm_q, self.norm_k = RMSNorm(dim, eps=eps), RMSNorm(dim, eps=eps)
        self.has_image_input = False

    def context_kv(self, ctx2: torch.Tensor, fold: bool = True, pad_n: Optional[int] = None):
        m = 1
        if fold and ctx2.is_cuda and ops._OPT["fold_pad_keys"]:
            n = pad_run(ctx2) if pad_n is None else pad_n
            if ctx2.shape[0] - n >= 2 and n + 1 < ops.VT_MIN_KV:
                m = ctx2.shape[0] - n
                ctx2 = ctx2[: n + 1]
        cin = QuantizedInput(ctx2) if getattr(self.k, "_gf_w8", None) is not None else ctx2
        k, v = linear(cin, self.k), linear(cin, self.v)
        ops.rmsnorm_rope(k, self.norm_k.weight, None, None, self.head_dim, self.norm_k.eps)
        return k, v, m

    def attend(self, x2, kv):
        q = linear(x2, self.q)
        ops.rmsnorm_rope(q, self.norm_q.weight, None, None, self.head_dim, self.norm_q.eps)
        return ops.flash_attn(q, kv[0], kv[1], self.num_heads, last_key_mult=kv[2] if len(kv) > 2 else 1)

    FOLD_K_MAX = 2560

    def fold_ok(self, kv) -> bool:
        if not ops._OPT["fold_cross_o"] or torch.is_grad_enabled() or len(kv) < 3 or kv[2] == 1 or self.head_dim != 128:
            return False
        if getattr(self.o, "_gf_w8", None) is not None:
            return False
        n = kv[0].shape[0]
        k = self.num_heads * self.fold_pad(n)
        return n <= ops.CROSS_FOLD_MAX_KEYS and k <= self.FOLD_K_MAX and k % 64 == 0

    @staticmethod
    def fold_pad(n_keys: int) -> int:
        return -(-(n_keys + 1) // 16) * 16

    def fold_table(self, kv):
        return ops.cross_fold_table(kv[1], self.o.weight, self.num_heads, self.fold_pad(kv[0].shape[0]))

    def attend_probs(self, x2, kv):
        q = linear(x2, self.q)
        ops.rmsnorm_rope(q, self.norm_q.weight, None, None, self.head_dim, self.norm_q.eps)
        return ops.cross_probs(q, kv[0], self.num_heads, self.fold_pad(kv[0].shape[0]), last_key_mult=kv[2])

    def forward(self, x: torch.Tensor, y: torch.Tensor):
        x2 = _tokens2d(x)
        a = self.attend(x2, self.context_kv(_tokens2d(y)))
        return linear(a, self.o).view(x.shape)


class GateModule(nn.Module):

    def forward(self, x, gate, residual):
        if x.shape != residual.shape:
            raise GoalForceError("GateModule: x and residual must have the same shape")
        d = x.shape[-1]
        g = gate.reshape(-1, d)
        if x.dim() == 3 and g.shape[0] == x.shape[0] and x.shape[0] > 1:
            return torch.stack([ops.gate_residual(x[b], g[b].contiguous(), residual[b]) for b in range(x.shape[0])])
        if g.shape[0] != 1:
            raise GoalForceError("GateModule: gate must be [B or 1, 1, D] (per-token gates are outside the Goal-Force path)")
        return ops.gate_residual(x, g[0].contiguous(), residual)


class DiTBlock(nn.Module):

    def __init__(self, has_image_input: bool, dim: int, num_heads: int, ffn_dim: int, eps: float = 1e-6):
        super().__init__()
        self.dim, self.num_heads, self.ffn_dim, self.eps = dim, num_heads, ffn_dim, eps
        self.self_attn = SelfAttention(dim, num_heads, eps)
        self.cross_attn = CrossAttention(dim, num_heads, eps, has_image_input=has_image_input)
        self.norm1 = nn.LayerNorm(dim, eps=eps, elementwise_affine=False)
        self.norm2 = nn.LayerNorm(dim, eps=eps, elementwise_affine=False)
        self.norm3 = nn.LayerNorm(dim, eps=eps)
        self.ffn = nn.Sequential(nn.Linear(dim, ffn_dim), nn.GELU(approximate="tanh"), nn.Linear(ffn_dim, dim))
        self.modulation = nn.Parameter(torch.randn(1, 6, dim) / dim ** 0.5)
        self.gate = GateModule()

    def forward(self, x, context, t_mod, freqs, context_kv=None, out=None, sp=None, keep=None, self_attn_memo=None,
                fold_pad_keys=True, pad_n=None):
        if t_mod.dim() == 4:
            raise NotImplementedError("per-token t_mod (seperated_timestep) is outside the Goal-Force path")
        x2 = _tokens2d(x)
        rope = _as_rope(freqs, x.device)
        mod = ops.modulation(self.modulation, t_mod.contiguous(), onep_mask=0b010010)
        fp8 = getattr(self.ffn[0], "_gf_w8", None) is not None
        if self_attn_memo is not None and "x" in self_attn_memo:
            x_new = self_attn_memo.pop("x")
            ev = self_attn_memo.pop("ev", None)
            if ev is not None:
                torch.cuda.current_stream(x_new.device).wait_event(ev)
                x_new.record_stream(torch.cuda.current_stream(x_new.device))
            if out is not None:
                x_new = out.copy_(x_new)
            h = None if fp8 else torch.empty_like(x2)
        else:
            if fp8:
                h = QuantizedInput.layernorm(x2, scale1p=mod[1], shift=mod[0], eps=self.eps)
            else:
                h = ops.layernorm_modulate(x2, scale1p=mod[1], shift=mod[0], eps=self.eps)
            a = self.self_attn.attend(h, rope, sp, keep)
            x_new = out if out is not None else torch.empty_like(x2)
            linear(a, self.self_attn.o, epilogue=ops.EPI_BIAS_GATE_RESID, resid=x2, gate=mod[2], out=x_new)
            if keep is not None and keep.get("wide"):
                keep["x1"] = x_new.clone()
            if self_attn_memo is not None:
                self_attn_memo["x"] = x_new.clone()
                if x_new.is_cuda:
                    self_attn_memo["ev"] = torch.cuda.Event()
                    self_attn_memo["ev"].record(torch.cuda.current_stream(x_new.device))
        if fp8:
            h = QuantizedInput.layernorm(x_new, weight=self.norm3.weight, bias=self.norm3.bias, eps=self.eps)
        else:
            ops.layernorm_modulate(x_new, weight=self.norm3.weight, bias=self.norm3.bias, eps=self.eps, out=h)
        if context_kv is None:
            context_kv = self.cross_attn.context_kv(_tokens2d(context), fold=fold_pad_keys and keep is None, pad_n=pad_n)
        ca = self.cross_attn
        if keep is None and not fp8 and ca.fold_ok(context_kv):
            u = context_kv[3] if len(context_kv) > 3 else ca.fold_table(context_kv)
            ops.gemm(ca.attend_probs(h, context_kv), u, ca.o.bias, epilogue=ops.EPI_BIAS_RESID, resid=x_new, out=x_new)
        else:
            a = ca.attend(h, context_kv)
            linear(a, ca.o, epilogue=ops.EPI_BIAS_RESID, resid=x_new, out=x_new)
        if keep is not None and keep.get("wide"):
            keep["x2b"] = x_new.clone()
# ... 132 lines not shown
```

### goal_force_amd/ops.py

```python
from __future__ import annotations

import math

import torch

from . import _lib
from ._lib import (EPI_BIAS, EPI_BIAS_GATE_RESID, EPI_BIAS_GELU_TANH, EPI_BIAS_MUL, EPI_BIAS_RESID, EPI_BIAS_SILU,
                   GoalForceError)

__all__ = [
    "modulation", "layernorm_modulate", "rmsnorm_rope", "gate_residual", "gemm", "flash_attn", "patchify_im2col", "unpatchify",
    "cfg_euler_step", "act", "add", "sub", "rel_l1", "force_map",
    "EPI_BIAS", "EPI_BIAS_GELU_TANH", "EPI_BIAS_GATE_RESID", "EPI_BIAS_RESID", "EPI_BIAS_SILU", "EPI_BIAS_MUL",
]

_BF16 = torch.bfloat16
_FP8 = torch.float8_e4m3fn

PROFILE_ATTN = None
PROFILE_GEMM = None
PROFILE_CONV = None


def _stream(t: torch.Tensor):
# ... 67 lines not shown
            raise GoalForceError(f"{op}: {' / '.join(tensors)} must be contiguous and equal-sized")
    return n


def kv_pad(skv: int) -> int:
    return -(-skv // 64) * 64


class _timed:
    __slots__ = ("prof", "what", "e0")

    def __init__(self, prof, *what):
        self.prof, self.what = prof, what

    def __enter__(self):
        if self.prof is not None:
            self.e0 = torch.cuda.Event(enable_timing=True)
            self.e0.record()

    def __exit__(self, exc_type, *exc):
        if self.prof is not None and exc_type is None:
            e1 = torch.cuda.Event(enable_timing=True)
            e1.record()
            self.prof.append((self.e0, e1) + self.what)
        return False


def _linear_operands(a, w, scale):
    if scale is None:
        _req(a, "linear: activation")
        av, M, K, lda = _rows2d(a, "linear: activation")
        N, ldw = _weight(w, "linear: weight", K)
    else:
        _mat(a, "fp8 linear: activation", _FP8)
        av, (M, K), lda = a, a.shape, a.stride(0)
        N, ldw = _weight(w, "fp8 linear: weight", K, _FP8)
        _vec(scale, "fp8 linear: row scale", M, torch.float32)
    return av, M, K, lda, N, ldw


def modulation(param, t, onep_mask: int):
    _req(param, "modulation.param")
    _req(t, "modulation.t")
    dim = param.shape[-1]
    k = param.numel() // dim
    t_rows = t.numel() // dim
    if not param.is_contiguous() or not t.is_contiguous() or t.shape[-1] != dim:
        raise GoalForceError("modulation: param/t must be contiguous with equal last dim")
    out = torch.empty((k, dim), dtype=_BF16, device=param.device)
    _lib.check(_lib.load().gf_modulation(_ptr(param), _ptr(t), _ptr(out), k, dim, t_rows, int(onep_mask),
                                         _stream(param)), "gf_modulation")
    return out


def layernorm_modulate(x, weight=None, bias=None, scale1p=None, shift=None, eps=1e-6, out=None):
    _req(x, "layernorm_modulate.x")
    xv, rows, dim, xs = _rows2d(x, "layernorm_modulate.x")
    if out is None:
        out = torch.empty(x.shape, dtype=_BF16, device=x.device)
    ov, _, _, os_ = _rows2d(out, "layernorm_modulate.out")
    _vec(weight, "layernorm_modulate.weight", dim)
    _vec(bias, "layernorm_modulate.bias", dim)
    _vec(scale1p, "layernorm_modulate.scale1p", dim)
    _vec(shift, "layernorm_modulate.shift", dim)
    _lib.check(_lib.load().gf_layernorm_modulate(_ptr(xv), _ptr(ov), _ptr(weight), _ptr(bias), _ptr(scale1p),
                                                 _ptr(shift), rows, dim, xs, os_, float(eps), _stream(x)),
               "gf_layernorm_modulate")
    return out


def rmsnorm_rope(x, weight, cos=None, sin=None, head_dim=128, eps=1e-6):
    _req(x, "rmsnorm_rope.x")
    _req(weight, "rmsnorm_rope.weight")
    xv, rows, dim, xs = _rows2d(x, "rmsnorm_rope.x")
    if cos is not None:
        _req(cos, "rmsnorm_rope.cos", torch.float32)
        _req(sin, "rmsnorm_rope.sin", torch.float32)
        if cos.shape != (rows, head_dim // 2) or sin.shape != cos.shape or not cos.is_contiguous() \
                or not sin.is_contiguous():
            raise GoalForceError(f"rmsnorm_rope: cos/sin must be contiguous [{rows}, {head_dim // 2}]")
    _lib.check(_lib.load().gf_rmsnorm_rope(_ptr(xv), _ptr(weight), _ptr(cos), _ptr(sin), rows, dim, head_dim, xs,
                                           float(eps), _stream(x)), "gf_rmsnorm_rope")
    return x


def modulate(x, shift, scale):
    _req(x, "modulate.x")
    xv, rows, dim, xs = _rows2d(x, "modulate.x")
    _vec(shift, "modulate.shift", dim, required=True)
    _vec(scale, "modulate.scale", dim, required=True)
    out = torch.empty(x.shape, dtype=_BF16, device=x.device)
    ov, _, _, os_ = _rows2d(out, "modulate.out")
    _lib.check(_lib.load().gf_modulate(_ptr(xv), _ptr(ov), _ptr(scale), _ptr(shift), rows, dim, xs, os_, _stream(x)), "gf_modulate")
    return out


def gate_residual(x, gate, residual):
    _req(x, "gate_residual.x")
    _req(residual, "gate_residual.residual")
    xv, rows, dim, xs = _rows2d(x, "gate_residual.x")
    rv, rrows, rdim, rs = _rows2d(residual, "gate_residual.residual")
    if (rrows, rdim) != (rows, dim):
        raise GoalForceError(f"gate_residual: residual must match x [{rows}, {dim}]")
    _vec(gate, "gate_residual.gate", dim, required=True)
    out = torch.empty(x.shape, dtype=_BF16, device=x.device)
    ov, _, _, os_ = _rows2d(out, "gate_residual.out")
    _lib.check(_lib.load().gf_gate_residual(_ptr(xv), _ptr(gate), _ptr(rv), _ptr(ov), rows, dim, xs, rs, os_, _stream(x)),
               "gf_gate_residual")
    return out


def rope_apply(x, cos, sin, head_dim):
    _req(x, "rope_apply.x")
    xv, rows, dim, xs = _rows2d(x, "rope_apply.x")
    for n, t in (("cos", cos), ("sin", sin)):
        _req(t, f"rope_apply.{n}", torch.float32)
        if tuple(t.shape) != (rows, head_dim // 2) or not t.is_contiguous():
            raise GoalForceError(f"rope_apply.{n}: expected contiguous [{rows}, {head_dim // 2}] fp32")
    out = torch.empty(x.shape, dtype=_BF16, device=x.device)
    ov, _, _, os_ = _rows2d(out, "rope_apply.out")
    _lib.check(_lib.load().gf_rope_apply(_ptr(xv), _ptr(ov), _ptr(cos), _ptr(sin), rows, dim, head_dim, xs, os_, _stream(x)),
               "gf_rope_apply")
    return out


def _gemm(a, w, row_scale, bias, epilogue, resid, gate, out):
    av, M, K, lda, N, ldw = _linear_operands(a, w, row_scale)
    if out is None:
        out = torch.empty(a.shape[:-1] + (N,), dtype=_BF16, device=a.device)
    ov, Mo, No, ldc = _rows2d(out, "gemm[_fp8].out")
    if (Mo, No) != (M, N):
        raise GoalForceError(f"gemm[_fp8].out: expected [{M}, {N}], got [{Mo}, {No}]")
    ldr = 0
    if resid is not None:
        _req(resid, "gemm[_fp8].resid")
        resid, Mr, Nr, ldr = _rows2d(resid, "gemm[_fp8].resid")
        if (Mr, Nr) != (M, N):
            raise GoalForceError(f"gemm[_fp8].resid: expected [{M}, {N}], got [{Mr}, {Nr}]")
    _vec(gate, "gemm[_fp8].gate", N)
    _vec(bias, "gemm[_fp8].bias", N)
    lib = _lib.load()
    fn, scale = (lib.gf_gemm_bf16, ()) if row_scale is None else (lib.gf_gemm_fp8, (_ptr(row_scale),))
    with _timed(PROFILE_GEMM, M, N, K, int(epilogue)):
        _lib.check(fn(_ptr(av), lda, _ptr(w), ldw, *scale, _ptr(bias), _ptr(ov), ldc, M, N, K, int(epilogue), _ptr(resid), ldr,
                      _ptr(gate), _stream(a)), fn.__name__)
    return out


def gemm(a, w, bias=None, epilogue=EPI_BIAS, resid=None, gate=None, out=None):
    return _gemm(a, w, None, bias, epilogue, resid, gate, out)


VT_MIN_KV = 2048
_LIB_DEFAULTS = {"prefer_8wave": 0, "a4_stagger": 2, "a4_group_m": 0, "conv_nb": 0, "conv_gather": 0, "conv_direct": 1, "vae_rms3": 1}
_OPT = {"attn_k3": True, "vt_from_gemm": True, "conv_padded": True, "fold_pad_keys": True, "attn_q_prescale": True, "vae_attn_offset": True,
        "fold_cross_o": True}


def lib_option(name: str) -> int:
    import ctypes
    v = ctypes.c_int(0)
    _lib.check(_lib.load().gf_get_option(name.encode(), ctypes.byref(v)), f"gf_get_option({name})")
    return int(v.value)


class options:

    def __init__(self, **kv):
        for k in kv:
            if k not in _OPT and k not in _LIB_DEFAULTS:
                raise GoalForceError(f"ops.options: unknown option {k!r}")
        self.kv, self.old = kv, {}

    @staticmethod
    def _apply_one(k, v):
        if k in _OPT:
            _OPT[k] = bool(v)
        else:
            _lib.check(_lib.load().gf_set_option(k.encode(), int(v)), f"gf_set_option({k})")

    def __enter__(self):
        self.old = {}
        try:
            for k, v in self.kv.items():
                old = _OPT[k] if k in _OPT else lib_option(k)
                self._apply_one(k, v)
                self.old[k] = old
        except BaseException:
            self.__exit__(None, None, None)
            raise
        return self

    def __exit__(self, *exc):
        for k, v in reversed(list(self.old.items())):
            self._apply_one(k, v)
        self.old = {}
        return False


_VT_WS = {}


def _vt_workspace(numel, device):
    key = (device.index, torch.cuda.current_stream(device).cuda_stream)
    ws = _VT_WS.get(key)
    if ws is None or ws.numel() < numel:
        ws = _VT_WS[key] = torch.empty((numel,), dtype=_BF16, device=device)
    return ws


def _vt_shape(skv, num_heads, head_dim):
    return skv >= VT_MIN_KV and head_dim == 128 and num_heads * 128 * kv_pad(skv) < 2 ** 31


def vt32_ok(skv, num_heads, head_dim):
    return _vt_shape(skv, num_heads, head_dim) and _OPT["attn_k3"] and _OPT["vt_from_gemm"]


def _linear_vt32(x, w, x_scale, bias):
    xv, skv, K, ldx, N, ldw = _linear_operands(x, w, x_scale)
    _vec(bias, "linear_vt32[_fp8].bias", N)
    vt = _vt_workspace(N * kv_pad(skv), x.device)
    lib = _lib.load()
    fn, scale = (lib.gf_linear_vt32, ()) if x_scale is None else (lib.gf_linear_vt32_fp8, (_ptr(x_scale),))
    _lib.check(fn(_ptr(xv), ldx, *scale, _ptr(w), ldw, _ptr(bias), _ptr(vt), skv, kv_pad(skv), N, K, _stream(x)), fn.__name__)
    return vt


def linear_vt32(x, weight, bias):
    return _linear_vt32(x, weight, None, bias)


def linear_vt32_fp8(x8, x_scale, w8, bias):
    if x_scale is None:
        raise GoalForceError("linear_vt32_fp8.x_scale: required")
    return _linear_vt32(x8, w8, x_scale, bias)


def _vt_attn(lib, q, k, v, vt, out, lse, sq, skv, num_heads, head_dim, scale, k3):
    tr, fa = (lib.gf_transpose_v32, lib.gf_flash_attn_fwd_vt32) if k3 else (lib.gf_transpose_v, lib.gf_flash_attn_fwd_vt)
    if vt is None:
        vt = _vt_workspace(num_heads * 128 * kv_pad(skv), q.device)
        _lib.check(tr(_ptr(v), v.stride(0), _ptr(vt), skv, kv_pad(skv), num_heads, _stream(q)), "gf_transpose_v")
    _lib.check(fa(_ptr(q), _ptr(k), _ptr(vt), _ptr(out), _ptr(lse), sq, skv, kv_pad(skv), num_heads, head_dim,
                  q.stride(0), k.stride(0), out.stride(0), float(scale), _stream(q)), "gf_flash_attn_fwd_vt")


def flash_attn(q, k, v, num_heads, out=None, scale=None, vt=None, last_key_mult=1, finished_q=False):
    for n, t in (("q", q), ("k", k)) + ((("v", v),) if vt is None else ()):
        _mat(t, f"flash_attn.{n}")
    sq, hd_all = q.shape
    skv = k.shape[0]
    head_dim = hd_all // num_heads
    if k.shape[1] != hd_all or (vt is None and v.shape != k.shape) or head_dim * num_heads != hd_all:
        raise GoalForceError("flash_attn: q/k/v shape mismatch")
    if vt is not None and not vt32_ok(skv, num_heads, head_dim):
        raise GoalForceError("flash_attn: a pre-transposed V is only taken by kernel 3 (key length >= VT_MIN_KV, head_dim 128)")
    if out is None:
        out = torch.empty((sq, hd_all), dtype=_BF16, device=q.device)
    if scale is None:
        scale = 1.0 / math.sqrt(head_dim)
    if last_key_mult != 1 and (vt is not None or skv >= VT_MIN_KV):
        raise GoalForceError("flash_attn: last_key_mult is for short key sequences (the text context), not the V^T path")
    long_keys = _vt_shape(skv, num_heads, head_dim)
    if finished_q and vt is not None:
        raise GoalForceError("flash_attn: finished_q goes to kernel 2, which does not take kernel 3's V^T operand")
    if vt is not None and vt.numel() < num_heads * 128 * kv_pad(skv):
        raise GoalForceError("flash_attn.vt: buffer smaller than heads*128*kv_pad")
    lib = _lib.load()
    with _timed(PROFILE_ATTN, sq, skv, num_heads):
        if long_keys:
            _vt_attn(lib, q, k, v, vt, out, None, sq, skv, num_heads, head_dim, scale, _OPT["attn_k3"] and not finished_q)
        elif last_key_mult != 1:
            _lib.check(lib.gf_flash_attn_fwd_lastmult(_ptr(q), _ptr(k), _ptr(v), _ptr(out), sq, skv, num_heads, head_dim, q.stride(0),
                                                      k.stride(0), v.stride(0), out.stride(0), float(scale), float(last_key_mult),
                                                      _stream(q)), "gf_flash_attn_fwd_lastmult")
        else:
            _lib.check(lib.gf_flash_attn_fwd(_ptr(q), _ptr(k), _ptr(v), _ptr(out), sq, skv, num_heads, head_dim,
                                             q.stride(0), k.stride(0), v.stride(0), out.stride(0), float(scale),
                                             _stream(q)), "gf_flash_attn_fwd")
    return out


SAGE_T, SAGE_TAU, SAGE_E = 128, 0, 8
SAGE_QBLK, SAGE_KBLK = 32, 64
_SAGE_WS = {}
_SAGE_SCRATCH_PER_HEAD = 64 * 128 * 8


def _sage_rows(t, name, num_heads):
    _mat(t, name)
    if t.shape[1] != num_heads * 128:
        raise GoalForceError(f"{name}: {t.shape[1]} columns for {num_heads} heads: the sage backend is built for head_dim 128")
    if t.shape[0] < 1:
        raise GoalForceError(f"{name}: empty sequence")
    if t.stride(0) % 8 or t.data_ptr() % 16:
        raise GoalForceError(f"{name}: row stride must be a multiple of 8 elements and the data 16-byte aligned")
    return t.shape[0], t.stride(0)


def _sage_scale(scale):
    scale = 1.0 / math.sqrt(128) if scale is None else float(scale)
    if not (0.0 < scale < math.inf):
        raise GoalForceError(f"sage attention: the softmax scale must be positive and finite, got {scale}")
    return scale


def _sage_scratch(num_heads, device):
    return torch.empty((num_heads * _SAGE_SCRATCH_PER_HEAD,), dtype=torch.uint8, device=device)


def sage_k_mean(k, num_heads):
    skv, ldk = _sage_rows(k, "sage_k_mean.k", num_heads)
    mu = torch.empty((num_heads, 128), dtype=torch.float32, device=k.device)
    _lib.check(_lib.load().gf_sage_k_mean(_ptr(k), ldk, _ptr(mu), _ptr(_sage_scratch(num_heads, k.device)), skv, num_heads, _stream(k)),
               "gf_sage_k_mean")
    return mu


def sage_quant_q(q, num_heads):
    sq, ldq = _sage_rows(q, "sage_quant_q.q", num_heads)
    q8 = torch.empty((sq, num_heads * 128), dtype=torch.int8, device=q.device)
    sc = torch.empty((num_heads, -(-sq // SAGE_QBLK)), dtype=torch.float32, device=q.device)
    _lib.check(_lib.load().gf_sage_quant_q(_ptr(q), ldq, _ptr(q8), _ptr(sc), sq, num_heads, _stream(q)), "gf_sage_quant_q")
    return q8, sc


def sage_quant_k(k, num_heads, mu=None):
    skv, ldk = _sage_rows(k, "sage_quant_k.k", num_heads)
    if mu is None:
        mu = sage_k_mean(k, num_heads)
    _vec(mu, "sage_quant_k.mu", num_heads * 128, torch.float32)
    kv_pad8 = -(-skv // SAGE_T) * SAGE_T
    k8 = torch.empty((kv_pad8, num_heads * 128), dtype=torch.int8, device=k.device)
    sc = torch.empty((num_heads, kv_pad8 // SAGE_KBLK), dtype=torch.float32, device=k.device)
    _lib.check(_lib.load().gf_sage_quant_k(_ptr(k), ldk, _ptr(mu), _ptr(k8), _ptr(sc), skv, num_heads, _stream(k)), "gf_sage_quant_k")
    return k8, sc, mu


def sage_quant_vt(v, num_heads, vt=None, kv_len=None):
    if vt is None:
        skv, ldv = _sage_rows(v, "sage_quant_vt.v", num_heads)
        src, vt_in = v, 0
    else:
        _req(vt, "sage_quant_vt.vt")
        if kv_len is None or kv_len < 1:
            raise GoalForceError("sage_quant_vt: a V^T input needs kv_len")
        skv, ldv, src, vt_in = kv_len, kv_pad(kv_len), vt, 1
        if vt.numel() < num_heads * 128 * ldv:
            raise GoalForceError("sage_quant_vt.vt: buffer smaller than heads*128*kv_pad")
    kv_pad8 = -(-skv // SAGE_T) * SAGE_T
    vt8 = torch.empty((num_heads * 128, kv_pad8), dtype=torch.uint8, device=src.device)
    sc = torch.empty((num_heads, 128), dtype=torch.float32, device=src.device)
    _lib.check(_lib.load().gf_sage_quant_vt(_ptr(src), ldv, vt_in, _ptr(vt8), _ptr(sc), _ptr(_sage_scratch(num_heads, src.device)), skv,
                                            num_heads, _stream(src)), "gf_sage_quant_vt")
    return vt8, sc


def sage_attn_quantized(q8, q_scale, k8, k_scale, vt8, v_scale, kv_len, num_heads, scale=None, out=None):
    sq = q8.shape[0]
    scale = _sage_scale(scale)
    if out is None:
        out = torch.empty((sq, num_heads * 128), dtype=_BF16, device=q8.device)
    _lib.check(_lib.load().gf_sage_attn_fwd(_ptr(q8), _ptr(q_scale), _ptr(k8), _ptr(k_scale), _ptr(vt8), _ptr(v_scale), _ptr(out),
                                            out.stride(0), sq, kv_len, num_heads, scale, _stream(q8)), "gf_sage_attn_fwd")
    return out


def sage_attn(q, k, v, num_heads, scale=None, vt=None, out=None):
    scale = _sage_scale(scale)
    sq, ldq = _sage_rows(q, "sage_attn.q", num_heads)
    skv, ldk = _sage_rows(k, "sage_attn.k", num_heads)
    if vt is None:
        sv, ldv = _sage_rows(v, "sage_attn.v", num_heads)
        if sv != skv:
            raise GoalForceError(f"sage_attn: k has {skv} keys, v {sv}")
        src, vt_in = v, 0
    else:
        _req(vt, "sage_attn.vt")
        ldv, src, vt_in = kv_pad(skv), vt, 1
        if vt.numel() < num_heads * 128 * ldv:
            raise GoalForceError("sage_attn.vt: buffer smaller than heads*128*kv_pad")
    out = _out(out, "sage_attn.out", sq, num_heads * 128, q.device)
    if out.stride(0) % 8:
        raise GoalForceError("sage_attn.out: row stride must be a multiple of 8 elements")
    lib = _lib.load()
    nbytes = int(lib.gf_sage_workspace_bytes(sq, skv, num_heads))
    key = (q.device.index, torch.cuda.current_stream(q.device).cuda_stream)
    ws = _SAGE_WS.get(key)
    if ws is None or ws.numel() < nbytes:
        ws = _SAGE_WS[key] = torch.empty((nbytes,), dtype=torch.uint8, device=q.device)
    with _timed(PROFILE_ATTN, sq, skv, num_heads):
        _lib.check(lib.gf_sage_attn(_ptr(q), ldq, _ptr(k), ldk, _ptr(src), ldv, vt_in, _ptr(out), out.stride(0), sq, skv, num_heads,
                                    scale, _ptr(ws), _stream(q)), "gf_sage_attn")
    return out


CROSS_FOLD_MAX_KEYS = 63


def cross_probs(q, k, num_heads, n_pad, last_key_mult=1, scale=None, out=None):
    _mat(q, "cross_probs.q")
    _mat(k, "cross_probs.k")
    sq, hd_all = q.shape
    n_keys = k.shape[0]
    head_dim = hd_all // num_heads
    if k.shape[1] != hd_all or head_dim * num_heads != hd_all:
        raise GoalForceError("cross_probs: q/k shape mismatch")
    out = _out(out, "cross_probs.out", sq, num_heads * n_pad, q.device)
    if scale is None:
        scale = 1.0 / math.sqrt(head_dim)
    _lib.check(_lib.load().gf_cross_probs(_ptr(q), _ptr(k), _ptr(out), sq, n_keys, n_pad, num_heads, head_dim, q.stride(0), k.stride(0),
                                          out.stride(0), float(scale), float(last_key_mult), _stream(q)), "gf_cross_probs")
    return out


def cross_fold_table(v, w_o, num_heads, n_pad):
    _mat(v, "cross_fold_table.v")
    n_keys, hd_all = v.shape
    N, ldw = _weight(w_o, "cross_fold_table.w_o", hd_all)
    if hd_all % num_heads:
        raise GoalForceError(f"cross_fold_table: {hd_all} columns do not divide into {num_heads} heads")
    u = torch.empty((N, num_heads * n_pad), dtype=_BF16, device=v.device)
    _lib.check(_lib.load().gf_cross_fold_table(_ptr(v), _ptr(w_o), _ptr(u), n_keys, n_pad, num_heads, hd_all // num_heads, N, v.stride(0),
                                               ldw, u.stride(0), _stream(v)), "gf_cross_fold_table")
    return u


def flash_attn_lse(q, k, v, num_heads, scale=None):
    for n, t in (("q", q), ("k", k), ("v", v)):
        _mat(t, f"flash_attn_lse.{n}")
    sq, hd_all = q.shape
    skv = k.shape[0]
    head_dim = hd_all // num_heads
    if k.shape[1] != hd_all or v.shape != k.shape or head_dim * num_heads != hd_all:
        raise GoalForceError("flash_attn_lse: q/k/v shape mismatch")
    if scale is None:
        scale = 1.0 / math.sqrt(head_dim)
    out = torch.empty((sq, hd_all), dtype=_BF16, device=q.device)
    lse = torch.empty((sq, num_heads), dtype=torch.float32, device=q.device)
    lib = _lib.load()
    if _vt_shape(skv, num_heads, head_dim):
        _vt_attn(lib, q, k, v, None, out, lse, sq, skv, num_heads, head_dim, scale, _OPT["attn_k3"])
        return out, lse
    _lib.check(lib.gf_flash_attn_fwd_lse(_ptr(q), _ptr(k), _ptr(v), _ptr(out), _ptr(lse), sq, skv, num_heads, head_dim,
                                         q.stride(0), k.stride(0), v.stride(0), out.stride(0), float(scale),
                                         _stream(q)), "gf_flash_attn_fwd_lse")
    return out, lse


def flash_attn_bwd(q, k, v, o, dout, lse, num_heads, scale=None, need_dkv=True):
    for n, t in (("q", q), ("k", k), ("v", v), ("o", o), ("dout", dout)):
        _mat(t, f"flash_attn_bwd.{n}")
    sq, hd_all = q.shape
    skv = k.shape[0]
    head_dim = hd_all // num_heads
    if scale is None:
        scale = 1.0 / math.sqrt(head_dim)
    if lse.dtype != torch.float32 or tuple(lse.shape) != (sq, num_heads) or not lse.is_contiguous():
        raise GoalForceError("flash_attn_bwd.lse: expected contiguous fp32 [Sq, heads]")
    dq = torch.empty_like(q, memory_format=torch.contiguous_format)
    dk = torch.empty((skv, hd_all), dtype=_BF16, device=q.device) if need_dkv else None
    dv = torch.empty((skv, hd_all), dtype=_BF16, device=q.device) if need_dkv else None
    lib = _lib.load()
    ws = torch.empty((int(lib.gf_flash_attn_bwd_workspace_bytes(sq, skv, num_heads)),), dtype=torch.uint8, device=q.device)
    _lib.check(lib.gf_flash_attn_bwd(_ptr(q), _ptr(k), _ptr(v), _ptr(o), _ptr(dout), _ptr(lse), _ptr(ws), _ptr(dq),
                                             _ptr(dk) if need_dkv else None, _ptr(dv) if need_dkv else None, sq, skv, num_heads, head_dim,
                                             q.stride(0), k.stride(0), v.stride(0), o.stride(0), dout.stride(0), dq.stride(0),
                                             dk.stride(0) if need_dkv else hd_all, dv.stride(0) if need_dkv else hd_all, float(scale),
                                             _stream(q)), "gf_flash_attn_bwd")
    return dq, dk, dv


def patchify_im2col(src0, src1=None, kpad=None):
    _req(src0, "patchify.src0")
    if src0.dim() != 4 or not src0.is_contiguous():
        raise GoalForceError("patchify.src0: expected contiguous [c,F,H,W]")
    c0, F, H, W = src0.shape
    c1 = 0
    if src1 is not None:
        _req(src1, "patchify.src1")
        if src1.dim() != 4 or not src1.is_contiguous() or src1.shape[1:] != src0.shape[1:]:
            raise GoalForceError("patchify.src1: expected contiguous [c1,F,H,W] matching src0")
        c1 = src1.shape[0]
    if kpad is None:
        kpad = -(-((c0 + c1) * 4) // 64) * 64
    out = torch.empty((F * (H // 2) * (W // 2), kpad), dtype=_BF16, device=src0.device)
    _lib.check(_lib.load().gf_patchify_im2col(_ptr(src0), c0, _ptr(src1), c1, _ptr(out), F, H, W, kpad,
                                              _stream(src0)), "gf_patchify_im2col")
    return out


def unpatchify(tokens, c, f, h, w):
    _req(tokens, "unpatchify.tokens")
# ... 450 lines not shown
```

### include/goalforce.h

```cpp
#ifndef GOALFORCE_H
#define GOALFORCE_H

#include <stdint.h>

#if defined(GF_BUILD)
#define GF_API __attribute__((visibility("default")))
#else
#define GF_API
#endif

#ifdef __cplusplus
extern "C" {
#endif

typedef enum {
    GF_OK = 0,
    GF_ERR_INVALID_ARG = -1,
    GF_ERR_UNSUPPORTED = -2,
    GF_ERR_LAUNCH = -3
} gf_status;

GF_API const char* gf_version(void);
GF_API const char* gf_last_error(void);
#define GF_ABI_VERSION 20
GF_API int gf_abi_version(void);
GF_API int gf_set_option(const char* name, int value);
GF_API int gf_get_option(const char* name, int* value);
GF_API void gf_reset_options(void);

GF_API int gf_layernorm_modulate(const void* x, void* out, const void* weight, const void* bias,
                          const void* scale1p, const void* shift,
                          int64_t rows, int64_t dim, int64_t x_stride, int64_t out_stride,
                          float eps, void* stream);

GF_API int gf_modulation(const void* param, const void* t, void* out, int64_t k, int64_t dim,
                         int64_t t_rows, uint32_t onep_mask, void* stream);

GF_API int gf_rmsnorm_rope(void* x, const void* weight, const float* cos_tab, const float* sin_tab,
                    int64_t rows, int64_t dim, int64_t head_dim, int64_t x_stride,
                    float eps, void* stream);

typedef enum {
    GF_EPI_BIAS = 0,
    GF_EPI_BIAS_GELU_TANH = 1,
    GF_EPI_BIAS_GATE_RESID = 2,
    GF_EPI_BIAS_RESID = 3,
    GF_EPI_BIAS_SILU = 4,
    GF_EPI_BIAS_MUL = 5
} gf_epilogue;

GF_API int gf_gemm_bf16(const void* A, int64_t lda, const void* W, int64_t ldw, const void* bias,
                 void* C, int64_t ldc, int64_t M, int64_t N, int64_t K,
                 int epilogue, const void* resid, int64_t ldr, const void* gate,
                 void* stream);

GF_API int gf_gemm_bf16_batched(const void* A, int64_t lda, int64_t strideA, const void* W, int64_t ldw, int64_t strideW, void* C,
                                int64_t ldc, int64_t strideC, int64_t M, int64_t N, int64_t K, int64_t batch, void* stream);

GF_API int gf_flash_attn_fwd(const void* q, const void* k, const void* v, void* o,
                      int64_t q_len, int64_t kv_len, int64_t heads, int64_t head_dim,
                      int64_t q_stride, int64_t k_stride, int64_t v_stride, int64_t o_stride,
                      float scale, void* stream);

GF_API int gf_transpose_v(const void* v, int64_t v_stride, void* vt, int64_t kv_len, int64_t kv_pad, int64_t heads, void* stream);
GF_API int gf_flash_attn_fwd_vt(const void* q, const void* k, const void* vt, void* o, float* lse,
                         int64_t q_len, int64_t kv_len, int64_t kv_pad, int64_t heads, int64_t head_dim,
                         int64_t q_stride, int64_t k_stride, int64_t o_stride, float scale, void* stream);

GF_API int gf_transpose_v32(const void* v, int64_t v_stride, void* vt, int64_t kv_len, int64_t kv_pad, int64_t heads, void* stream);
GF_API int gf_flash_attn_fwd_vt32(const void* q, const void* k, const void* vt, void* o, float* lse,
                                  int64_t q_len, int64_t kv_len, int64_t kv_pad, int64_t heads, int64_t head_dim,
                                  int64_t q_stride, int64_t k_stride, int64_t o_stride, float scale, void* stream);

GF_API int gf_linear_vt32(const void* x, int64_t ldx, const void* w, int64_t ldw, const void* bias, void* vt,
                          int64_t kv_len, int64_t kv_pad, int64_t N, int64_t K, void* stream);

GF_API int gf_flash_attn_fwd_lastmult(const void* q, const void* k, const void* v, void* o, int64_t q_len, int64_t kv_len,
                                      int64_t heads, int64_t head_dim, int64_t q_stride, int64_t k_stride, int64_t v_stride,
                                      int64_t o_stride, float scale, float last_key_multiplicity, void* stream);

GF_API int gf_cross_probs(const void* q, const void* k, void* p, int64_t q_len, int64_t n_keys, int64_t n_pad, int64_t heads,
                          int64_t head_dim, int64_t q_stride, int64_t k_stride, int64_t p_stride, float scale,
                          float last_key_multiplicity, void* stream);

GF_API int gf_cross_fold_table(const void* v, const void* w_o, void* u, int64_t n_keys, int64_t n_pad, int64_t heads, int64_t head_dim,
                               int64_t n_out, int64_t v_stride, int64_t w_stride, int64_t u_stride, void* stream);

GF_API int gf_flash_attn_fwd_lse(const void* q, const void* k, const void* v, void* o, float* lse,
                          int64_t q_len, int64_t kv_len, int64_t heads, int64_t head_dim,
                          int64_t q_stride, int64_t k_stride, int64_t v_stride, int64_t o_stride,
                          float scale, void* stream);
GF_API int64_t gf_flash_attn_bwd_workspace_bytes(int64_t q_len, int64_t kv_len, int64_t heads);
GF_API int gf_flash_attn_bwd(const void* q, const void* k, const void* v, const void* o, const void* dout,
                      const float* lse, void* workspace, void* dq, void* dk, void* dv,
                      int64_t q_len, int64_t kv_len, int64_t heads, int64_t head_dim,
                      int64_t q_stride, int64_t k_stride, int64_t v_stride, int64_t o_stride, int64_t do_stride,
                      int64_t dq_stride, int64_t dk_stride, int64_t dv_stride, float scale, void* stream);

GF_API int gf_layernorm_bwd(const void* x, int64_t x_stride, const void* dy, int64_t dy_stride, const void* g, void* dx,
                            int64_t dx_stride, float* dg_acc, float* db_acc, int64_t rows, int64_t dim, float eps, void* stream);
GF_API int gf_rmsnorm_rope_bwd(const void* x, int64_t x_stride, const void* dy, int64_t dy_stride, const void* weight,
                               const float* cos_tab, const float* sin_tab, void* dx, int64_t dx_stride, float* dw_acc,
                               int64_t rows, int64_t dim, int64_t head_dim, float eps, void* stream);
GF_API int gf_colsum(const void* a, int64_t lda, const void* b, int64_t ldb, const void* gate, void* out, int64_t ldo,
                     float* acc, int64_t rows, int64_t cols, void* stream);
GF_API int gf_act_bwd(const void* u, const void* df, void* du, int64_t n, int kind, void* stream);
GF_API int gf_mse_loss(const void* pred, const void* target, void* dpred, float* loss, int64_t n, float weight, void* stream);
GF_API int gf_adamw_step(void* param, const void* grad, float* exp_avg, float* exp_avg_sq, int64_t n, float lr, float beta1,
                         float beta2, float eps, float weight_decay, int64_t step, float grad_scale, void* stream);
GF_API int gf_f32_to_bf16(const float* src, void* dst, int64_t n, void* stream);
GF_API int gf_sumsq(const void* x, int64_t n, float* acc, void* stream);

GF_API int gf_patchify_im2col(const void* src0, int64_t c0, const void* src1, int64_t c1,
                       void* out, int64_t F, int64_t H, int64_t W, int64_t kpad, void* stream);

GF_API int gf_unpatchify(const void* tokens, void* out, int64_t c, int64_t f, int64_t h, int64_t w,
                  void* stream);

GF_API int gf_cfg_euler_step(void* latents, const void* posi, const void* nega,
                      float cfg_scale, float dsigma, int64_t n, void* stream);

GF_API int gf_act(const void* x, void* out, int64_t n, int kind, void* stream);

GF_API int gf_add_bf16(const void* a, const void* b, void* out, int64_t n, void* stream);

GF_API int gf_sub_bf16(const void* a, const void* b, void* out, int64_t n, void* stream);
GF_API int gf_rel_l1_bf16(const void* cur, const void* prev, int64_t n, void* sums, void* stream);

GF_API int gf_force_map(void* out, int64_t frames, int64_t H, int64_t W,
                 const int32_t* channels, const float* params, const float* centers,
                 int64_t n_blobs, int clamp01, void* stream);


GF_API int gf_vae_prep_latent(const void* z, int64_t sc, int64_t st, int64_t sy, int64_t sx,
                              const void* mean, const void* inv_std, void* out,
                              int64_t C, int64_t T, int64_t H, int64_t W, int64_t cpad, void* stream);

GF_API int gf_vae_im2col(const void* src, const void* cache, void* out, int64_t T_out, int64_t H, int64_t W,
                         int64_t C, int64_t kt, int64_t ks, int mode, int64_t t_stride, int64_t t_off,
                         int64_t kpad, void* stream);

GF_API int gf_conv3d_bf16(const void* src, const void* cache, const void* Wm, int64_t ldw, const void* bias,
                          void* out, int64_t ldc, int64_t T_in, int64_t T_out, int64_t H, int64_t W, int64_t C,
                          int kt, int ks, int mode, int t_stride, int t_off, int64_t N, int64_t K, int epilogue,
                          const void* resid, int64_t ldr, void* stream);

GF_API int gf_vae_finish_latent(const void* x, int64_t ldx, const void* mean, const void* inv_std, void* out,
                                int64_t rows, int64_t C, void* stream);

GF_API int gf_vae_rmsnorm_silu(const void* x, const void* gamma, void* out, int64_t rows, int64_t C,
                               int silu, void* stream);

GF_API int gf_softmax_rows(const void* x, int64_t ldx, const void* bias, int64_t ldb, void* out, int64_t ldo,
                           int64_t rows, int64_t ncols, int64_t nvalid, float scale, void* stream);

GF_API int gf_rowmax_neg_bf16(const void* x, int64_t ldx, void* out, int64_t ldo, int64_t rows, int64_t ncols, void* stream);

GF_API int gf_transpose_pad(const void* src, int64_t ld_src, void* dst, int64_t R, int64_t C, int64_t rpad,
                            void* stream);

GF_API int gf_transpose_pad_batched(const void* src, int64_t ld_src, int64_t stride_src, void* dst, int64_t stride_dst, int64_t R,
                                    int64_t C, int64_t rpad, int64_t batch, void* stream);

GF_API int gf_vae_tile_blend(void* values, void* weight, const void* tile, int64_t nch, int64_t T, int64_t th,
                             int64_t tw, int64_t tc, int64_t H, int64_t W, int64_t y0, int64_t x0,
                             int top, int bottom, int left, int right, int64_t border_h, int64_t border_w,
// ... 62 lines not shown
```

Baseline: 0.6152.

## Fuse Q RMSNorm+RoPE into projection GEMM epilogue and attention prologue

The Q projection GEMM gets a new epilogue that also emits per-row, per-128-column partial sums of squares. The flash-attention kernel 3 and the cross-probs kernel gain a QN template variant that applies the RMSNorm scale, weight and (for self-attention) RoPE to the Q fragments right after loading them. This removes a separate norm/rope pass that reads and writes the full Q tensor in HBM. The cost is extra per-thread work and table loads in the attention prologue, plus a new option flag (fuse_q_norm) and a GEMM path pinned to the a4 kernel.

```diff
diff --git a/goal_force_amd/csrc/gf_attention.hip b/goal_force_amd/csrc/gf_attention.hip
--- a/goal_force_amd/csrc/gf_attention.hip
+++ b/goal_force_amd/csrc/gf_attention.hip
@@ -1,4 +1,5 @@
 #include "gf_common.h"
+#include "gf_qnorm.h"
 #include <cstdlib>
 #include <type_traits>
 
@@ -26,6 +27,15 @@
     const u16* vt;
     long kv_pad;
     float last_key_bias;
+};
+
+struct AttnQNorm {
+    const float* sumsq = nullptr;
+    const u16* weight = nullptr;
+    const float* cos = nullptr;
+    const float* sin = nullptr;
+    int nseg = 0;
+    float inv_dim = 0.f, eps = 0.f;
 };
 
 constexpr int AT2_THREADS = 512;
@@ -478,8 +488,8 @@
     acc = __builtin_amdgcn_mfma_f32_16x16x32_bf16(a, b, acc, 0, 0, 0);
 }
 
-template <int NQ>
-__global__ __launch_bounds__(At3<NQ>::THREADS, (NQ == 2 ? 2 : 1)) void flash_attn_fwd_kernel3(const AttnArgs p) {
+template <int NQ, bool QN = false>
+__global__ __launch_bounds__(At3<NQ>::THREADS, (NQ == 2 ? 2 : 1)) void flash_attn_fwd_kernel3(const AttnArgs p, const AttnQNorm qn) {
     constexpr int NP = At3<NQ>::PIECES, NW = At3<NQ>::WAVES, RW = At3<NQ>::ROWS, NS = At3<NQ>::SLOTS;
     extern __shared__ __attribute__((aligned(16))) char smem[];
     GF_LDS char* lds = (GF_LDS char*)smem;
@@ -798,6 +808,21 @@
 
     stage(0, 0, 0);
     if (nt > 1) stage(0, 1, 1);
+    if constexpr (QN) {
+#pragma unroll
+        for (int qb = 0; qb < NQ; ++qb) {
+            const long qr = min(q0 + 16 * qb + r, p.q_len - 1);
+            const float rstd = gf_qnorm_rstd(qn.sumsq + qr * qn.nseg, qn.nseg, qn.inv_dim, qn.eps);
+            const u16* wp = qn.weight + head * HD + 8 * g;
+            const float* cp = qn.cos + qr * (HD / 2) + 4 * g;
+            const float* sp = qn.sin + qr * (HD / 2) + 4 * g;
+#pragma unroll
+            for (int ks = 0; ks < 4; ++ks)
+                qf[qb][ks] = __builtin_bit_cast(
+                    bf16x8, gf_qnorm_apply8<true>(__builtin_bit_cast(u16x8, qf[qb][ks]), rstd, *reinterpret_cast<const u16x8*>(wp + 32 * ks),
+                                                  *reinterpret_cast<const f32x4*>(cp + 16 * ks), *reinterpret_cast<const f32x4*>(sp + 16 * ks)));
+        }
+    }
 #pragma unroll
     for (int qb = 0; qb < NQ; ++qb)
 #pragma unroll
@@ -1060,9 +1085,9 @@
     return GF_OK;
 }
 
-extern "C" GF_API int gf_flash_attn_fwd_vt32(const void* q, const void* k, const void* vt, void* o, float* lse, int64_t q_len,
-                                             int64_t kv_len, int64_t kv_pad, int64_t heads, int64_t head_dim, int64_t q_stride,
-                                             int64_t k_stride, int64_t o_stride, float scale, void* stream) {
+static int flash_attn_fwd_vt32_impl(const void* q, const void* k, const void* vt, void* o, float* lse, int64_t q_len, int64_t kv_len,
+                                    int64_t kv_pad, int64_t heads, int64_t head_dim, int64_t q_stride, int64_t k_stride, int64_t o_stride,
+                                    float scale, void* stream, const AttnQNorm* qn) {
     GF_CHECK_ARG(q && k && vt && o, "gf_flash_attn_fwd_vt32: null pointer");
     if (head_dim != HD) {
         gf_set_error("gf_flash_attn_fwd_vt32: head_dim=%ld unsupported (kernel is built for 128)", (long)head_dim);
@@ -1080,7 +1105,10 @@
     if (q_len == 0) return GF_OK;
     static GfDeviceOnce once;
     hipError_t e = gf_once_per_device(once, [] {
-        return hipFuncSetAttribute(reinterpret_cast<const void*>(flash_attn_fwd_kernel3<K3_NQ>),
+        hipError_t r = hipFuncSetAttribute(reinterpret_cast<const void*>(flash_attn_fwd_kernel3<K3_NQ, false>),
+                                           hipFuncAttributeMaxDynamicSharedMemorySize, AT3_LDS);
+        if (r != hipSuccess) return r;
+        return hipFuncSetAttribute(reinterpret_cast<const void*>(flash_attn_fwd_kernel3<K3_NQ, true>),
                                    hipFuncAttributeMaxDynamicSharedMemorySize, AT3_LDS);
     });
     if (e != hipSuccess) {
@@ -1106,8 +1134,39 @@
     a.kv_pad = kv_pad;
     a.dbg = nullptr;
     a.last_key_bias = 0.f;
-    hipLaunchKernelGGL(flash_attn_fwd_kernel3<K3_NQ>, dim3((unsigned)(a.n_qblocks * a.heads)), dim3(At3<K3_NQ>::THREADS), AT3_LDS,
-                       (hipStream_t)stream, a);
+    if (qn)
+        hipLaunchKernelGGL((flash_attn_fwd_kernel3<K3_NQ, true>), dim3((unsigned)(a.n_qblocks * a.heads)), dim3(At3<K3_NQ>::THREADS), AT3_LDS,
+                           (hipStream_t)stream, a, *qn);
+    else
+        hipLaunchKernelGGL((flash_attn_fwd_kernel3<K3_NQ, false>), dim3((unsigned)(a.n_qblocks * a.heads)), dim3(At3<K3_NQ>::THREADS), AT3_LDS,
+                           (hipStream_t)stream, a, AttnQNorm{});
     GF_CHECK_LAUNCH("gf_flash_attn_fwd_vt32");
     return GF_OK;
 }
+
+extern "C" GF_API int gf_flash_attn_fwd_vt32(const void* q, const void* k, const void* vt, void* o, float* lse, int64_t q_len,
+                                             int64_t kv_len, int64_t kv_pad, int64_t heads, int64_t head_dim, int64_t q_stride,
+                                             int64_t k_stride, int64_t o_stride, float scale, void* stream) {
+    return flash_attn_fwd_vt32_impl(q, k, vt, o, lse, q_len, kv_len, kv_pad, heads, head_dim, q_stride, k_stride, o_stride, scale, stream,
+                                    nullptr);
+}
+
+extern "C" GF_API int gf_flash_attn_fwd_qnorm(const void* q, const float* q_sumsq, const void* norm_weight, const float* cos_tab,
+                                              const float* sin_tab, float eps, const void* k, const void* vt, void* o, float* lse,
+                                              int64_t q_len, int64_t kv_len, int64_t kv_pad, int64_t heads, int64_t head_dim,
+                                              int64_t q_stride, int64_t k_stride, int64_t o_stride, float scale, void* stream) {
+    GF_CHECK_ARG(q_sumsq && norm_weight && cos_tab && sin_tab, "gf_flash_attn_fwd_qnorm: null q_sumsq / norm_weight / cos / sin");
+    GF_CHECK_ARG(gf_aligned16(q_sumsq) && gf_aligned16(norm_weight) && gf_aligned16(cos_tab) && gf_aligned16(sin_tab),
+                 "gf_flash_attn_fwd_qnorm: 16-byte alignment required");
+    GF_CHECK_ARG(heads > 0 && heads <= GF_QN_MAXSEG, "gf_flash_attn_fwd_qnorm: heads=%ld (the row has heads segments, <= %d)", (long)heads,
+                 GF_QN_MAXSEG);
+    AttnQNorm qn;
+    qn.sumsq = q_sumsq;
+    qn.weight = (const u16*)norm_weight;
+    qn.cos = cos_tab;
+    qn.sin = sin_tab;
+    qn.nseg = (int)heads;
+    qn.inv_dim = 1.0f / (float)(heads * HD);
+    qn.eps = eps;
+    return flash_attn_fwd_vt32_impl(q, k, vt, o, lse, q_len, kv_len, kv_pad, heads, head_dim, q_stride, k_stride, o_stride, scale, stream, &qn);
+}
diff --git a/goal_force_amd/csrc/gf_cross_fold.hip b/goal_force_amd/csrc/gf_cross_fold.hip
--- a/goal_force_amd/csrc/gf_cross_fold.hip
+++ b/goal_force_amd/csrc/gf_cross_fold.hip
@@ -1,4 +1,5 @@
 #include "gf_common.h"
+#include "gf_qnorm.h"
 
 namespace {
 
@@ -11,9 +12,17 @@
     acc = __builtin_amdgcn_mfma_f32_32x32x16_bf16(a, b, acc, 0, 0, 0);
 }
 
+struct CrossQNorm {
+    const float* sumsq;
+    const u16* weight;
+    int nseg;
+    float inv_dim, eps;
+};
+
+template <bool QN>
 __global__ __launch_bounds__(CF_THREADS) void cross_probs_kernel(const u16* __restrict__ q, const u16* __restrict__ k, u16* __restrict__ pout,
                                                                  int q_len, int n_keys, int n_pad, int heads, long q_stride, long k_stride,
-                                                                 long p_stride, float c, float last_key_bias) {
+                                                                 long p_stride, float c, float last_key_bias, const CrossQNorm qn) {
     __shared__ __attribute__((aligned(16))) char lds[CF_MAXK * 256];
     const int tid = threadIdx.x;
     const int lane = tid & 63, wave = tid >> 6;
@@ -38,6 +47,15 @@
         const u16* qp = q + (long)qr * q_stride + head * CF_HD + 8 * h;
 #pragma unroll
         for (int kd = 0; kd < 8; ++kd) qf[kd] = *reinterpret_cast<const bf16x8*>(qp + 16 * kd);
+        if constexpr (QN) {
+            const float rstd = gf_qnorm_rstd(qn.sumsq + (long)qr * qn.nseg, qn.nseg, qn.inv_dim, qn.eps);
+            const u16* wp = qn.weight + head * CF_HD + 8 * h;
+            const f32x4 z = {0.f, 0.f, 0.f, 0.f};
+#pragma unroll
+            for (int kd = 0; kd < 8; ++kd)
+                qf[kd] = __builtin_bit_cast(bf16x8, gf_qnorm_apply8<false>(__builtin_bit_cast(u16x8, qf[kd]), rstd,
+                                                                           *reinterpret_cast<const u16x8*>(wp + 16 * kd), z, z));
+        }
     }
     __syncthreads();
 
@@ -156,9 +174,9 @@
 
 }
 
-extern "C" GF_API int gf_cross_probs(const void* q, const void* k, void* p, int64_t q_len, int64_t n_keys, int64_t n_pad, int64_t heads,
-                                     int64_t head_dim, int64_t q_stride, int64_t k_stride, int64_t p_stride, float scale,
-                                     float last_key_multiplicity, void* stream) {
+static int cross_probs_launch(const void* q, const void* k, void* p, int64_t q_len, int64_t n_keys, int64_t n_pad, int64_t heads,
+                              int64_t head_dim, int64_t q_stride, int64_t k_stride, int64_t p_stride, float scale,
+                              float last_key_multiplicity, void* stream, const CrossQNorm* qn) {
     GF_CHECK_ARG(q && k && p, "gf_cross_probs: null pointer");
     if (head_dim != CF_HD) {
         gf_set_error("gf_cross_probs: head_dim=%ld unsupported (kernel is built for 128)", (long)head_dim);
@@ -177,10 +195,34 @@
     const float c = scale * 1.4426950408889634f;
     const float bias = last_key_multiplicity != 1.0f ? log2f(last_key_multiplicity) / c : 0.f;
     const dim3 grid((unsigned)((q_len + CF_QB - 1) / CF_QB), (unsigned)heads);
-    hipLaunchKernelGGL(cross_probs_kernel, grid, dim3(CF_THREADS), 0, (hipStream_t)stream, (const u16*)q, (const u16*)k, (u16*)p,
-                       (int)q_len, (int)n_keys, (int)n_pad, (int)heads, (long)q_stride, (long)k_stride, (long)p_stride, c, bias);
+    if (qn)
+        hipLaunchKernelGGL(cross_probs_kernel<true>, grid, dim3(CF_THREADS), 0, (hipStream_t)stream, (const u16*)q, (const u16*)k, (u16*)p,
+                           (int)q_len, (int)n_keys, (int)n_pad, (int)heads, (long)q_stride, (long)k_stride, (long)p_stride, c, bias, *qn);
+    else
+        hipLaunchKernelGGL(cross_probs_kernel<false>, grid, dim3(CF_THREADS), 0, (hipStream_t)stream, (const u16*)q, (const u16*)k, (u16*)p,
+                           (int)q_len, (int)n_keys, (int)n_pad, (int)heads, (long)q_stride, (long)k_stride, (long)p_stride, c, bias,
+                           CrossQNorm{});
     GF_CHECK_LAUNCH("gf_cross_probs");
     return GF_OK;
+}
+
+extern "C" GF_API int gf_cross_probs(const void* q, const void* k, void* p, int64_t q_len, int64_t n_keys, int64_t n_pad, int64_t heads,
+                                     int64_t head_dim, int64_t q_stride, int64_t k_stride, int64_t p_stride, float scale,
+                                     float last_key_multiplicity, void* stream) {
+    return cross_probs_launch(q, k, p, q_len, n_keys, n_pad, heads, head_dim, q_stride, k_stride, p_stride, scale, last_key_multiplicity,
+                              stream, nullptr);
+}
+
+extern "C" GF_API int gf_cross_probs_qnorm(const void* q, const float* q_sumsq, const void* norm_weight, float eps, const void* k, void* p,
+                                           int64_t q_len, int64_t n_keys, int64_t n_pad, int64_t heads, int64_t head_dim, int64_t q_stride,
+                                           int64_t k_stride, int64_t p_stride, float scale, float last_key_multiplicity, void* stream) {
+    GF_CHECK_ARG(q_sumsq && norm_weight && gf_aligned16(q_sumsq) && gf_aligned16(norm_weight),
+                 "gf_cross_probs_qnorm: q_sumsq [q_len, heads] fp32 and norm_weight [heads*128] bf16, 16-byte aligned");
+    GF_CHECK_ARG(heads > 0 && heads <= GF_QN_MAXSEG, "gf_cross_probs_qnorm: heads=%ld (the row has heads segments, <= %d)", (long)heads,
+                 GF_QN_MAXSEG);
+    const CrossQNorm qn{q_sumsq, (const u16*)norm_weight, (int)heads, 1.0f / (float)(heads * CF_HD), eps};
+    return cross_probs_launch(q, k, p, q_len, n_keys, n_pad, heads, head_dim, q_stride, k_stride, p_stride, scale, last_key_multiplicity,
+                              stream, &qn);
 }
 
 extern "C" GF_API int gf_cross_fold_table(const void* v, const void* w_o, void* u, int64_t n_keys, int64_t n_pad, int64_t heads,
diff --git a/goal_force_amd/csrc/gf_gemm.hip b/goal_force_amd/csrc/gf_gemm.hip
--- a/goal_force_amd/csrc/gf_gemm.hip
+++ b/goal_force_amd/csrc/gf_gemm.hip
@@ -35,9 +35,9 @@
     long lda, ldw, ldc, ldr;
     long sA = 0, sW = 0, sC = 0;
     int tiles_m, tiles_n;
-    unsigned long long* rsv0 = nullptr;
+    float* sumsq = nullptr;
     ConvGeom cv;
-    int rsv1 = 0;
+    int nseg = 0;
     int stagger;
     int wrows;
     int stagger_rows;
@@ -46,6 +46,19 @@
 };
 
 constexpr int GF_EPI_VT32 = 6;
+constexpr int GF_EPI_BIAS_SUMSQ = 7;
+
+template <int CTRL>
+__device__ __forceinline__ float gf_dpp_row(float x) {
+    return __builtin_bit_cast(float, __builtin_amdgcn_update_dpp(0, __builtin_bit_cast(int, x), CTRL, 0xf, 0xf, true));
+}
+__device__ __forceinline__ float gf_row16_sum(float s) {
+    s += gf_dpp_row<0xB1>(s);
+    s += gf_dpp_row<0x4E>(s);
+    s += gf_dpp_row<0x141>(s);
+    s += gf_dpp_row<0x140>(s);
+    return s;
+}
 
 __device__ __forceinline__ void glds16(const void* g, GF_LDS char* l) {
     __builtin_amdgcn_global_load_lds((const GF_GLOBAL void*)g, (GF_LDS void*)l, 16, 0, 0);
@@ -817,6 +830,13 @@
             } else {
                 yv = *(GF_LDS u16x8*)(ep + row * 256 + ((cc ^ (row & 15)) << 4));
             }
+            if constexpr (EPI == GF_EPI_BIAS_SUMSQ) {
+                float s = bf2f(yv[0]) * bf2f(yv[0]);
+#pragma unroll
+                for (int e = 1; e < 8; ++e) s = __builtin_fmaf(bf2f(yv[e]), bf2f(yv[e]), s);
+                s = gf_row16_sum(s);
+                if (cc == 0 && m < p.M && n_ok) p.sumsq[(long)m * p.nseg + ((n0 + wn * 128) >> 7)] = s;
+            }
             if (m < p.M && n_ok) {
                 u16x8 o = yv;
                 if constexpr (HAS_R) {
@@ -835,6 +855,11 @@
     }
 }
 
+static bool gemm_a4_bf16_ok(long M, long K, long lda, long ldw) {
+    return gf_options().prefer_8wave.load(std::memory_order_relaxed) == 0 && M >= 512 && K % 64 == 0 &&
+           256L * lda * 2 + K * 2L < (1L << 31) && 256L * ldw * 2 + K * 2L < (1L << 31);
+}
+
 template <int EPI, bool FP8 = false>
 int launch_gemm_a4(const GemmArgs& a0, hipStream_t stream) {
     GemmArgs a = a0;
@@ -860,9 +885,7 @@
 int launch_gemm(const GemmArgs& a, hipStream_t stream) {
     const bool use_a4 = gf_options().prefer_8wave.load(std::memory_order_relaxed) == 0;
     if constexpr (!FP8) {
-        if (use_a4 && a.M >= 512 && a.K % 64 == 0 && 256L * a.lda * 2 + a.K * 2L < (1L << 31) &&
-            256L * a.ldw * 2 + a.K * 2L < (1L << 31))
-            return launch_gemm_a4<EPI>(a, stream);
+        if (gemm_a4_bf16_ok(a.M, a.K, a.lda, a.ldw)) return launch_gemm_a4<EPI>(a, stream);
     } else {
         if (use_a4 && a.M >= 512 && a.K % 128 == 0 && 256L * a.lda + a.K < (1L << 31) && 256L * a.ldw + a.K < (1L << 31))
             return launch_gemm_a4<EPI, true>(a, stream);
@@ -926,8 +949,8 @@
 
 static int gemm_dispatch(bool fp8, const void* A, int64_t lda, const void* W, int64_t ldw, const float* row_scale,
                          const void* bias, void* C, int64_t ldc, int64_t M, int64_t N, int64_t K, int epilogue,
-                         const void* resid, int64_t ldr, const void* gate, void* stream) {
-    const char* fn = fp8 ? "gf_gemm_fp8" : "gf_gemm_bf16";
+                         const void* resid, int64_t ldr, const void* gate, void* stream, float* sumsq = nullptr) {
+    const char* fn = sumsq ? "gf_gemm_bf16_sumsq" : fp8 ? "gf_gemm_fp8" : "gf_gemm_bf16";
     const int bke = fp8 ? 128 : 64, lal = fp8 ? 16 : 8;
     GF_CHECK_ARG(A && W && C, "%s: null A/W/C", fn);
     GF_CHECK_ARG(M >= 0 && N > 0 && K > 0, "%s: bad sizes M=%ld N=%ld K=%ld", fn, (long)M, (long)N, (long)K);
@@ -966,6 +989,11 @@
     a.wrows = (int)N;
     a.stagger_rows = 0;
     hipStream_t s = (hipStream_t)stream;
+    if (sumsq) {
+        a.sumsq = sumsq;
+        a.nseg = (int)(N / 128);
+        return launch_gemm_a4<GF_EPI_BIAS_SUMSQ>(a, s);
+    }
 #define GF_GEMM_CASE(E) case E: return fp8 ? launch_gemm<E, true>(a, s) : launch_gemm<E, false>(a, s);
     switch (epilogue) {
         GF_GEMM_CASE(GF_EPI_BIAS)
@@ -985,6 +1013,22 @@
                                    int64_t ldc, int64_t M, int64_t N, int64_t K, int epilogue, const void* resid,
                                    int64_t ldr, const void* gate, void* stream) {
     return gemm_dispatch(false, A, lda, W, ldw, nullptr, bias, C, ldc, M, N, K, epilogue, resid, ldr, gate, stream);
+}
+
+extern "C" GF_API int gf_gemm_bf16_sumsq_ok(int64_t M, int64_t N, int64_t K, int64_t lda, int64_t ldw) {
+    return N > 0 && N % 128 == 0 && K > 0 && gemm_a4_bf16_ok((long)M, (long)K, (long)lda, (long)ldw) ? 1 : 0;
+}
+
+extern "C" GF_API int gf_gemm_bf16_sumsq(const void* A, int64_t lda, const void* W, int64_t ldw, const void* bias, void* C, int64_t ldc,
+                                         float* sumsq, int64_t M, int64_t N, int64_t K, void* stream) {
+    GF_CHECK_ARG(sumsq && gf_aligned16(sumsq), "gf_gemm_bf16_sumsq: sumsq must be a 16-byte aligned [M, N/128] fp32 buffer");
+    GF_CHECK_ARG(N > 0 && N % 128 == 0, "gf_gemm_bf16_sumsq: N=%ld must be a multiple of 128 (whole head segments)", (long)N);
+    if (!gf_gemm_bf16_sumsq_ok(M, N, K, lda, ldw)) {
+        gf_set_error("gf_gemm_bf16_sumsq: M=%ld K=%ld is not a shape of the 4-wave kernel (M >= 512, K %% 64 == 0, option prefer_8wave "
+                     "off): ask gf_gemm_bf16_sumsq_ok first", (long)M, (long)K);
+        return GF_ERR_UNSUPPORTED;
+    }
+    return gemm_dispatch(false, A, lda, W, ldw, nullptr, bias, C, ldc, M, N, K, GF_EPI_BIAS, nullptr, 0, nullptr, stream, sumsq);
 }
 
 extern "C" GF_API int gf_gemm_fp8(const void* A8, int64_t lda, const void* W8, int64_t ldw, const float* row_scale,
diff --git a/goal_force_amd/csrc/gf_qnorm.h b/goal_force_amd/csrc/gf_qnorm.h
--- /dev/null
+++ b/goal_force_amd/csrc/gf_qnorm.h
@@ -0,0 +1,45 @@
+#pragma once
+#include "gf_common.h"
+
+constexpr int GF_QN_MAXSEG = 64;
+
+__device__ __forceinline__ float gf_qnorm_rstd(const float* __restrict__ part, int nseg, float inv_dim, float eps) {
+    float s = 0.f;
+    if ((nseg & 3) == 0) {
+        f32x4 v[GF_QN_MAXSEG / 4];
+#pragma unroll
+        for (int i = 0; i < GF_QN_MAXSEG / 4; ++i) v[i] = *reinterpret_cast<const f32x4*>(part + min(4 * i, nseg - 4));
+#pragma unroll
+        for (int i = 0; i < GF_QN_MAXSEG / 4; ++i) {
+            const bool in = 4 * i < nseg;
+#pragma unroll
+            for (int e = 0; e < 4; ++e) s += in ? v[i][e] : 0.f;
+        }
+    } else {
+        for (int i = 0; i < nseg; ++i) s += part[i];
+    }
+    return 1.0f / sqrtf(__builtin_fmaf(s, inv_dim, eps));
+}
+
+template <bool ROPE>
+__device__ __forceinline__ u16x8 gf_qnorm_apply8(const u16x8 v, const float rstd, const u16x8 w8, const f32x4 cs, const f32x4 sn) {
+    float y[8];
+#pragma unroll
+    for (int j = 0; j < 8; ++j) {
+        const float n = rbf(bf2f(v[j]) * rstd);
+        y[j] = rbf(n * bf2f(w8[j]));
+    }
+    u16x8 o;
+    if constexpr (ROPE) {
+#pragma unroll
+        for (int p = 0; p < 4; ++p) {
+            const float a = y[2 * p], b = y[2 * p + 1];
+            o[2 * p] = f2bf(__builtin_fmaf(a, cs[p], -(b * sn[p])));
+            o[2 * p + 1] = f2bf(__builtin_fmaf(a, sn[p], b * cs[p]));
+        }
+    } else {
+#pragma unroll
+        for (int j = 0; j < 8; ++j) o[j] = f2bf(y[j]);
+    }
+    return o;
+}
diff --git a/goal_force_amd/csrc/gf_rowops.hip b/goal_force_amd/csrc/gf_rowops.hip
--- a/goal_force_amd/csrc/gf_rowops.hip
+++ b/goal_force_amd/csrc/gf_rowops.hip
@@ -1,4 +1,5 @@
 #include "gf_common.h"
+#include "gf_qnorm.h"
 
 namespace {
 
@@ -344,6 +345,38 @@
             for (int j = 0; j < 8; ++j) o[j] = f2bf(y[j]);
         }
         *reinterpret_cast<u16x8*>(xr + i * 512) = o;
+    }
+}
+
+template <int NCH, bool ROPE>
+__global__ __launch_bounds__(64 * WROWS) void rmsnorm_rope_pre_wave_kernel(u16* __restrict__ x, const float* __restrict__ sumsq,
+                                                                             const u16* __restrict__ weight,
+                                                                             const float* __restrict__ cos_tab,
+                                                                             const float* __restrict__ sin_tab, long rows, int dim,
+                                                                             int head_dim, long x_stride, float inv_dim, float eps) {
+    const long row = (long)blockIdx.x * WROWS + (threadIdx.x >> 6);
+    if (row >= rows) return;
+    const int lane = threadIdx.x & 63;
+    const int nseg = dim >> 7;
+    u16* xr = x + row * x_stride;
+    const float rstd = gf_qnorm_rstd(sumsq + row * nseg, nseg, inv_dim, eps);
+    const int half = head_dim >> 1;
+    auto chunk = [&](int c0) __attribute__((always_inline)) {
+        const u16x8 v = *reinterpret_cast<const u16x8*>(xr + c0);
+        const u16x8 w8 = *reinterpret_cast<const u16x8*>(weight + c0);
+        f32x4 cs = {0.f, 0.f, 0.f, 0.f}, sn = {0.f, 0.f, 0.f, 0.f};
+        if constexpr (ROPE) {
+            const int p0 = (c0 % head_dim) >> 1;
+            cs = *reinterpret_cast<const f32x4*>(cos_tab + row * half + p0);
+            sn = *reinterpret_cast<const f32x4*>(sin_tab + row * half + p0);
+        }
+        *reinterpret_cast<u16x8*>(xr + c0) = gf_qnorm_apply8<ROPE>(v, rstd, w8, cs, sn);
+    };
+    if constexpr (NCH > 0) {
+#pragma unroll
+        for (int i = 0; i < NCH; ++i) chunk(i * 512 + lane * 8);
+    } else {
+        for (int c0 = lane * 8; c0 < dim; c0 += 512) chunk(c0);
     }
 }
 
@@ -628,3 +661,33 @@
     GF_CHECK_LAUNCH("gf_rmsnorm_rope");
     return GF_OK;
 }
+
+extern "C" GF_API int gf_rmsnorm_rope_pre(void* x, const float* sumsq, const void* weight, const float* cos_tab, const float* sin_tab,
+                                          int64_t rows, int64_t dim, int64_t head_dim, int64_t x_stride, float eps, void* stream) {
+    GF_CHECK_ARG(x && weight && sumsq, "gf_rmsnorm_rope_pre: null x/weight/sumsq");
+    GF_CHECK_ARG(rows >= 0 && dim > 0 && dim % 128 == 0 && dim <= GF_QN_MAXSEG * 128,
+                 "gf_rmsnorm_rope_pre: dim=%ld must be a multiple of 128 (whole segments of sumsq) and <= %d", (long)dim, GF_QN_MAXSEG * 128);
+    GF_CHECK_ARG((cos_tab == nullptr) == (sin_tab == nullptr), "gf_rmsnorm_rope_pre: cos/sin must both be set or both NULL");
+    GF_CHECK_ARG(head_dim > 0 && head_dim % 8 == 0 && dim % head_dim == 0,
+                 "gf_rmsnorm_rope_pre: head_dim=%ld must be a multiple of 8 dividing dim", (long)head_dim);
+    GF_CHECK_ARG(x_stride % 8 == 0 && x_stride >= dim && gf_aligned16(x) && gf_aligned16(weight) && gf_aligned16(sumsq) &&
+                     (!cos_tab || (gf_aligned16(cos_tab) && gf_aligned16(sin_tab))),
+                 "gf_rmsnorm_rope_pre: 16-byte alignment required");
+    if (rows == 0) return GF_OK;
+    const dim3 grid_((unsigned)((rows + WROWS - 1) / WROWS)), block_(64 * WROWS);
+    const float inv_dim = 1.0f / (float)dim;
+#define GF_RMS_PRE(NCH, ROPE)                                                                                            \
+    hipLaunchKernelGGL((rmsnorm_rope_pre_wave_kernel<NCH, ROPE>), grid_, block_, 0, (hipStream_t)stream, (u16*)x, sumsq, \
+                       (const u16*)weight, cos_tab, sin_tab, (long)rows, (int)dim, (int)head_dim, (long)x_stride, inv_dim, eps)
+#define GF_RMS_PRE_W(NCH)                                                                                                \
+    if (dim == NCH * 512 || NCH == 0) {                                                                                  \
+        if (cos_tab) GF_RMS_PRE(NCH, true);                                                                              \
+        else GF_RMS_PRE(NCH, false);                                                                                     \
+        GF_CHECK_LAUNCH("gf_rmsnorm_rope_pre");                                                                          \
+        return GF_OK;                                                                                                    \
+    }
+    GF_RMS_PRE_W(10) GF_RMS_PRE_W(8) GF_RMS_PRE_W(3) GF_RMS_PRE_W(0)
+#undef GF_RMS_PRE_W
+#undef GF_RMS_PRE
+    return GF_OK;
+}
diff --git a/goal_force_amd/dit.py b/goal_force_amd/dit.py
--- a/goal_force_amd/dit.py
+++ b/goal_force_amd/dit.py
@@ -135,6 +135,18 @@
         lin._gf_w8_key = param_key(lin.weight)
     q = x2 if isinstance(x2, QuantizedInput) else QuantizedInput(x2)
     return ops.gemm_fp8(q.x8, q.scale, w8, lin.bias, epilogue=epilogue, resid=resid, gate=gate, out=out)
+
+
+def linear_q(x2, lin: nn.Linear):
+    if getattr(lin, "_gf_w8", None) is None and not isinstance(x2, QuantizedInput) and ops.gemm_sumsq_ok(x2, lin.weight):
+        return ops.gemm_sumsq(x2, lin.weight, lin.bias)
+    return linear(x2, lin), None
+
+
+def norm_q(q, sumsq, weight, cos, sin, head_dim, eps):
+    if sumsq is None:
+        return ops.rmsnorm_rope(q, weight, cos, sin, head_dim, eps)
+    return ops.rmsnorm_rope_pre(q, sumsq, weight, cos, sin, head_dim, eps)
 
 
 def enable_fp8(module: nn.Module, enabled=True):
@@ -232,19 +244,26 @@
             ops.rmsnorm_rope(k, self.norm_k.weight, rope.cos, rope.sin, self.head_dim, self.norm_k.eps)
             hk = sp.heads_start(k, self.num_heads)
             hv = sp.heads_start(linear(xin, self.v), self.num_heads)
-            q = linear(xin, self.q)
-            ops.rmsnorm_rope(q, self.norm_q.weight, q_cos, q_sin, self.head_dim, self.norm_q.eps)
+            q, q_ss = self._project_q(xin)
+            norm_q(q, q_ss, self.norm_q.weight, q_cos, q_sin, self.head_dim, self.norm_q.eps)
             hq = sp.heads_start(q, self.num_heads)
             return sp.attention_started(hq, hk, hv, self.num_heads, tuple(q.shape), scale=attn_scale, backend="sage" if sage else "flash")
-        q, k = linear(xin, self.q), linear(xin, self.k)
+        (q, q_ss), k = self._project_q(xin), linear(xin, self.k)
         if keep is not None and keep.get("wide"):
             keep["qp"], keep["kp"] = q, k
             q, k = q.clone(), k.clone()
-        ops.rmsnorm_rope(q, self.norm_q.weight, q_cos, q_sin, self.head_dim, self.norm_q.eps)
+        one_gpu_bf16 = sp is None and keep is None and not fp8 and x2.is_cuda and self.v.weight.shape[0] >= 512 \
+            and ops.vt32_ok(x2.shape[0], self.num_heads, self.head_dim)
+        fuse_q = one_gpu_bf16 and q_ss is not None and not sage and ops._OPT["fuse_q_norm"]
+        if not fuse_q:
+            norm_q(q, q_ss, self.norm_q.weight, q_cos, q_sin, self.head_dim, self.norm_q.eps)
         ops.rmsnorm_rope(k, self.norm_k.weight, rope.cos, rope.sin, self.head_dim, self.norm_k.eps)
-        if sp is None and keep is None and not fp8 and x2.is_cuda and self.v.weight.shape[0] >= 512 \
-                and ops.vt32_ok(x2.shape[0], self.num_heads, self.head_dim):
-            return attn(q, k, None, self.num_heads, vt=ops.linear_vt32(x2, self.v.weight, self.v.bias), scale=attn_scale)
+        if one_gpu_bf16:
+            vt = ops.linear_vt32(x2, self.v.weight, self.v.bias)
+            if fuse_q:
+                return attn(q, k, None, self.num_heads, vt=vt, scale=attn_scale,
+                            qnorm=(q_ss, self.norm_q.weight, q_cos, q_sin, self.norm_q.eps))
+            return attn(q, k, None, self.num_heads, vt=vt, scale=attn_scale)
         if sp is None and keep is None and fp8 and xin.is_cuda and self.v.weight.shape[0] >= 512 and self.v.weight.shape[1] % 128 == 0 \
                 and ops.vt32_ok(xin.shape[0], self.num_heads, self.head_dim):
             if self.v._gf_w8_key != param_key(self.v.weight):
@@ -261,6 +280,9 @@
             return keep["attn"]
         return attn(q, k, v, self.num_heads, scale=attn_scale)
 
+    def _project_q(self, xin):
+        return linear_q(xin, self.q) if self.head_dim == 128 else (linear(xin, self.q), None)
+
     def forward(self, x, freqs):
         x2 = _tokens2d(x)
         a = self.attend(x2, _as_rope(freqs, x.device))
@@ -314,8 +336,11 @@
         return ops.cross_fold_table(kv[1], self.o.weight, self.num_heads, self.fold_pad(kv[0].shape[0]))
 
     def attend_probs(self, x2, kv):
-        q = linear(x2, self.q)
-        ops.rmsnorm_rope(q, self.norm_q.weight, None, None, self.head_dim, self.norm_q.eps)
+        q, q_ss = linear_q(x2, self.q)
+        if q_ss is not None and ops._OPT["fuse_q_norm"]:
+            return ops.cross_probs(q, kv[0], self.num_heads, self.fold_pad(kv[0].shape[0]), last_key_mult=kv[2],
+                                   qnorm=(q_ss, self.norm_q.weight, self.norm_q.eps))
+        norm_q(q, q_ss, self.norm_q.weight, None, None, self.head_dim, self.norm_q.eps)
         return ops.cross_probs(q, kv[0], self.num_heads, self.fold_pad(kv[0].shape[0]), last_key_mult=kv[2])
 
     def forward(self, x: torch.Tensor, y: torch.Tensor):
diff --git a/goal_force_amd/ops.py b/goal_force_amd/ops.py
--- a/goal_force_amd/ops.py
+++ b/goal_force_amd/ops.py
@@ -173,6 +173,36 @@
     _lib.check(_lib.load().gf_rmsnorm_rope(_ptr(xv), _ptr(weight), _ptr(cos), _ptr(sin), rows, dim, head_dim, xs,
                                            float(eps), _stream(x)), "gf_rmsnorm_rope")
     return x
+
+
+def rmsnorm_rope_pre(x, sumsq, weight, cos=None, sin=None, head_dim=128, eps=1e-6):
+    _req(x, "rmsnorm_rope_pre.x")
+    xv, rows, dim, xs = _rows2d(x, "rmsnorm_rope_pre.x")
+    _vec(weight, "rmsnorm_rope_pre.weight", dim, required=True)
+    _q_sumsq(sumsq, "rmsnorm_rope_pre.sumsq", rows, dim)
+    if (cos is None) != (sin is None):
+        raise GoalForceError("rmsnorm_rope_pre: cos and sin go together")
+    _rope_tables(cos, sin, "rmsnorm_rope_pre", rows, head_dim)
+    _lib.check(_lib.load().gf_rmsnorm_rope_pre(_ptr(xv), _ptr(sumsq), _ptr(weight), _ptr(cos), _ptr(sin), rows, dim, head_dim, xs,
+                                               float(eps), _stream(x)), "gf_rmsnorm_rope_pre")
+    return x
+
+
+def _q_sumsq(t, name: str, rows: int, dim: int):
+    if t is None:
+        raise GoalForceError(f"{name}: required")
+    _req(t, name, torch.float32)
+    if dim % 128 or tuple(t.shape) != (rows, dim // 128) or not t.is_contiguous():
+        raise GoalForceError(f"{name}: expected contiguous fp32 [{rows}, {dim}/128], got {tuple(t.shape)}")
+
+
+def _rope_tables(cos, sin, op: str, rows: int, head_dim: int):
+    for n, t in (("cos", cos), ("sin", sin)):
+        if t is None:
+            continue
+        _req(t, f"{op}.{n}", torch.float32)
+        if tuple(t.shape) != (rows, head_dim // 2) or not t.is_contiguous():
+            raise GoalForceError(f"{op}.{n}: expected contiguous [{rows}, {head_dim // 2}] fp32")
 
 
 def modulate(x, shift, scale):
@@ -242,10 +272,34 @@
     return _gemm(a, w, None, bias, epilogue, resid, gate, out)
 
 
+def gemm_sumsq_ok(a, w) -> bool:
+    if a.dtype != _BF16 or w.dtype != _BF16 or a.dim() < 1 or w.dim() != 2 or a.shape[-1] != w.shape[1]:
+        return False
+    av, M, K, lda = _rows2d(a, "gemm_sumsq_ok: activation")
+    return bool(_lib.load().gf_gemm_bf16_sumsq_ok(M, w.shape[0], K, lda, w.stride(0)))
+
+
+def gemm_sumsq(a, w, bias=None, out=None):
+    av, M, K, lda, N, ldw = _linear_operands(a, w, None)
+    if out is None:
+        out = torch.empty(a.shape[:-1] + (N,), dtype=_BF16, device=a.device)
+    ov, Mo, No, ldc = _rows2d(out, "gemm_sumsq.out")
+    if (Mo, No) != (M, N):
+        raise GoalForceError(f"gemm_sumsq.out: expected [{M}, {N}], got [{Mo}, {No}]")
+    if N % 128:
+        raise GoalForceError(f"gemm_sumsq: N={N} must be a multiple of 128")
+    _vec(bias, "gemm_sumsq.bias", N)
+    sumsq = torch.empty((M, N // 128), dtype=torch.float32, device=a.device)
+    with _timed(PROFILE_GEMM, M, N, K, int(EPI_BIAS)):
+        _lib.check(_lib.load().gf_gemm_bf16_sumsq(_ptr(av), lda, _ptr(w), ldw, _ptr(bias), _ptr(ov), ldc, _ptr(sumsq), M, N, K,
+                                                  _stream(a)), "gf_gemm_bf16_sumsq")
+    return out, sumsq
+
+
 VT_MIN_KV = 2048
 _LIB_DEFAULTS = {"prefer_8wave": 0, "a4_stagger": 2, "a4_group_m": 0, "conv_nb": 0, "conv_gather": 0, "conv_direct": 1, "vae_rms3": 1}
 _OPT = {"attn_k3": True, "vt_from_gemm": True, "conv_padded": True, "fold_pad_keys": True, "attn_q_prescale": True, "vae_attn_offset": True,
-        "fold_cross_o": True}
+        "fold_cross_o": True, "fuse_q_norm": True}
 
 
 def lib_option(name: str) -> int:
@@ -328,16 +382,22 @@
     return _linear_vt32(x8, w8, x_scale, bias)
 
 
-def _vt_attn(lib, q, k, v, vt, out, lse, sq, skv, num_heads, head_dim, scale, k3):
+def _vt_attn(lib, q, k, v, vt, out, lse, sq, skv, num_heads, head_dim, scale, k3, qnorm=None):
     tr, fa = (lib.gf_transpose_v32, lib.gf_flash_attn_fwd_vt32) if k3 else (lib.gf_transpose_v, lib.gf_flash_attn_fwd_vt)
     if vt is None:
         vt = _vt_workspace(num_heads * 128 * kv_pad(skv), q.device)
         _lib.check(tr(_ptr(v), v.stride(0), _ptr(vt), skv, kv_pad(skv), num_heads, _stream(q)), "gf_transpose_v")
+    if qnorm is not None:
+        sumsq, w, cos, sin, eps = qnorm
+        _lib.check(lib.gf_flash_attn_fwd_qnorm(_ptr(q), _ptr(sumsq), _ptr(w), _ptr(cos), _ptr(sin), float(eps), _ptr(k), _ptr(vt), _ptr(out),
+                                               _ptr(lse), sq, skv, kv_pad(skv), num_heads, head_dim, q.stride(0), k.stride(0),
+                                               out.stride(0), float(scale), _stream(q)), "gf_flash_attn_fwd_qnorm")
+        return
     _lib.check(fa(_ptr(q), _ptr(k), _ptr(vt), _ptr(out), _ptr(lse), sq, skv, kv_pad(skv), num_heads, head_dim,
                   q.stride(0), k.stride(0), out.stride(0), float(scale), _stream(q)), "gf_flash_attn_fwd_vt")
 
 
-def flash_attn(q, k, v, num_heads, out=None, scale=None, vt=None, last_key_mult=1, finished_q=False):
+def flash_attn(q, k, v, num_heads, out=None, scale=None, vt=None, last_key_mult=1, finished_q=False, qnorm=None):
     for n, t in (("q", q), ("k", k)) + ((("v", v),) if vt is None else ()):
         _mat(t, f"flash_attn.{n}")
     sq, hd_all = q.shape
@@ -358,10 +418,21 @@
         raise GoalForceError("flash_attn: finished_q goes to kernel 2, which does not take kernel 3's V^T operand")
     if vt is not None and vt.numel() < num_heads * 128 * kv_pad(skv):
         raise GoalForceError("flash_attn.vt: buffer smaller than heads*128*kv_pad")
+    k3 = _OPT["attn_k3"] and not finished_q
+    if qnorm is not None:
+        if not (long_keys and k3):
+            raise GoalForceError("flash_attn.qnorm: the fused q norm exists in kernel 3 only (key length >= VT_MIN_KV, head_dim 128, "
+                                 "attn_k3 on, no finished_q): use rmsnorm_rope_pre")
+        sumsq, w, cos, sin, _ = qnorm
+        _q_sumsq(sumsq, "flash_attn.qnorm.sumsq", sq, hd_all)
+        _vec(w, "flash_attn.qnorm.weight", hd_all, required=True)
+        if cos is None or sin is None:
+            raise GoalForceError("flash_attn.qnorm: cos and sin are required")
+        _rope_tables(cos, sin, "flash_attn.qnorm", sq, head_dim)
     lib = _lib.load()
     with _timed(PROFILE_ATTN, sq, skv, num_heads):
         if long_keys:
-            _vt_attn(lib, q, k, v, vt, out, None, sq, skv, num_heads, head_dim, scale, _OPT["attn_k3"] and not finished_q)
+            _vt_attn(lib, q, k, v, vt, out, None, sq, skv, num_heads, head_dim, scale, k3, qnorm)
         elif last_key_mult != 1:
             _lib.check(lib.gf_flash_attn_fwd_lastmult(_ptr(q), _ptr(k), _ptr(v), _ptr(out), sq, skv, num_heads, head_dim, q.stride(0),
                                                       k.stride(0), v.stride(0), out.stride(0), float(scale), float(last_key_mult),
@@ -490,7 +561,7 @@
 CROSS_FOLD_MAX_KEYS = 63
 
 
-def cross_probs(q, k, num_heads, n_pad, last_key_mult=1, scale=None, out=None):
+def cross_probs(q, k, num_heads, n_pad, last_key_mult=1, scale=None, out=None, qnorm=None):
     _mat(q, "cross_probs.q")
     _mat(k, "cross_probs.k")
     sq, hd_all = q.shape
@@ -501,6 +572,14 @@
     out = _out(out, "cross_probs.out", sq, num_heads * n_pad, q.device)
     if scale is None:
         scale = 1.0 / math.sqrt(head_dim)
+    if qnorm is not None:
+        sumsq, w, eps = qnorm
+        _q_sumsq(sumsq, "cross_probs.qnorm.sumsq", sq, hd_all)
+        _vec(w, "cross_probs.qnorm.weight", hd_all, required=True)
+        _lib.check(_lib.load().gf_cross_probs_qnorm(_ptr(q), _ptr(sumsq), _ptr(w), float(eps), _ptr(k), _ptr(out), sq, n_keys, n_pad,
+                                                    num_heads, head_dim, q.stride(0), k.stride(0), out.stride(0), float(scale),
+                                                    float(last_key_mult), _stream(q)), "gf_cross_probs_qnorm")
+        return out
     _lib.check(_lib.load().gf_cross_probs(_ptr(q), _ptr(k), _ptr(out), sq, n_keys, n_pad, num_heads, head_dim, q.stride(0), k.stride(0),
                                           out.stride(0), float(scale), float(last_key_mult), _stream(q)), "gf_cross_probs")
     return out
diff --git a/include/goalforce.h b/include/goalforce.h
--- a/include/goalforce.h
+++ b/include/goalforce.h
@@ -54,6 +54,13 @@
                  int epilogue, const void* resid, int64_t ldr, const void* gate,
                  void* stream);
 
+GF_API int gf_gemm_bf16_sumsq_ok(int64_t M, int64_t N, int64_t K, int64_t lda, int64_t ldw);
+GF_API int gf_gemm_bf16_sumsq(const void* A, int64_t lda, const void* W, int64_t ldw, const void* bias, void* C, int64_t ldc,
+                              float* sumsq, int64_t M, int64_t N, int64_t K, void* stream);
+
+GF_API int gf_rmsnorm_rope_pre(void* x, const float* sumsq, const void* weight, const float* cos_tab, const float* sin_tab,
+                               int64_t rows, int64_t dim, int64_t head_dim, int64_t x_stride, float eps, void* stream);
+
 GF_API int gf_gemm_bf16_batched(const void* A, int64_t lda, int64_t strideA, const void* W, int64_t ldw, int64_t strideW, void* C,
                                 int64_t ldc, int64_t strideC, int64_t M, int64_t N, int64_t K, int64_t batch, void* stream);
 
@@ -72,6 +79,11 @@
                                   int64_t q_len, int64_t kv_len, int64_t kv_pad, int64_t heads, int64_t head_dim,
                                   int64_t q_stride, int64_t k_stride, int64_t o_stride, float scale, void* stream);
 
+GF_API int gf_flash_attn_fwd_qnorm(const void* q, const float* q_sumsq, const void* norm_weight, const float* cos_tab,
+                                   const float* sin_tab, float eps, const void* k, const void* vt, void* o, float* lse,
+                                   int64_t q_len, int64_t kv_len, int64_t kv_pad, int64_t heads, int64_t head_dim,
+                                   int64_t q_stride, int64_t k_stride, int64_t o_stride, float scale, void* stream);
+
 GF_API int gf_linear_vt32(const void* x, int64_t ldx, const void* w, int64_t ldw, const void* bias, void* vt,
                           int64_t kv_len, int64_t kv_pad, int64_t N, int64_t K, void* stream);
 
@@ -82,6 +94,10 @@
 GF_API int gf_cross_probs(const void* q, const void* k, void* p, int64_t q_len, int64_t n_keys, int64_t n_pad, int64_t heads,
                           int64_t head_dim, int64_t q_stride, int64_t k_stride, int64_t p_stride, float scale,
                           float last_key_multiplicity, void* stream);
+
+GF_API int gf_cross_probs_qnorm(const void* q, const float* q_sumsq, const void* norm_weight, float eps, const void* k, void* p,
+                                int64_t q_len, int64_t n_keys, int64_t n_pad, int64_t heads, int64_t head_dim, int64_t q_stride,
+                                int64_t k_stride, int64_t p_stride, float scale, float last_key_multiplicity, void* stream);
 
 GF_API int gf_cross_fold_table(const void* v, const void* w_o, void* u, int64_t n_keys, int64_t n_pad, int64_t heads, int64_t head_dim,
                                int64_t n_out, int64_t v_stride, int64_t w_stride, int64_t u_stride, void* stream);
```

Measured after the change: 0.6149 (median of 2 runs). About the same (-0.1%).
